# MSNLAB/Federated-Lifelong-Person-ReID

Hardware: AMD Instinct MI355X
Metric: images/sec (whole node) per fed round, fedstil resnet50 (higher is better)
Workload: dtype bf16; 1 GPU; model=resnet50-fedstil, global_batch=64, img=128x64, images_per_round_per_client=512, num_classes=8000, lambda_k=2000, rehearsal_set=2000 exemplar budget + task (m=32/id), parallelism=fed-dp1 (1 client/GPU)

## Files before the change

flreid_amd/methods/common.py:

```python

from __future__ import annotations

import collections
import os
from typing import Any, Dict, List, Optional, Union

import torch
from torch.utils.data import DataLoader

from flreid_amd import ops
from flreid_amd.modules.client import ClientModule
from flreid_amd.modules.operator import OperatorModule
from flreid_amd.runtime.precision import autocast
from flreid_amd.tools.evaluate import calculate_similarity_distance, evaluate
from flreid_amd.tools.utils import model_on_device


def reset_optimizer_state_inplace(optimizer) -> None:
    import collections

    for state in optimizer.state.values():
        zeroed = True
        for k, v in state.items():
            if torch.is_tensor(v):
                v.zero_()
            elif isinstance(v, (int, float)):
                zeroed = False
        if not zeroed:
            optimizer.state = collections.defaultdict(dict)
            return


class BaseReIDOperator(OperatorModule):

    def set_optimizer_parameters(self, model, capturable: bool = False) -> None:
        defaults = dict(self.optimizer.defaults)
        if capturable and "capturable" in defaults:
            defaults["capturable"] = True
        params = [p for p in model.net.parameters() if p.requires_grad]
        for p in params:
            state = self.optimizer.state.get(p)
            if state and any(torch.is_tensor(v) and v.dim() > 0
                             and v.shape != p.shape for v in state.values()):
                del self.optimizer.state[p]
        group = {"params": params, **defaults}
        if capturable:
            group["capturable"] = True
        if (isinstance(self.optimizer, (torch.optim.Adam, torch.optim.AdamW))
                and params and params[0].is_cuda
                and os.environ.get("FLREID_FUSED_ADAM", "1") == "1"):
            group["fused"] = True
            group["foreach"] = False
        self.optimizer.param_groups = [group]

    def penalty(self, model) -> Optional[torch.Tensor]:
        return None

    def train_forward(self, model, data, target, **kwargs) -> Dict:
        score, feature = model.forward(data)
        loss = 0.0
        for loss_func in self.criterion:
            loss = loss + loss_func(score=score, feature=feature, target=target)
        return {"score": score, "feature": feature, "loss": loss}

    _invoke_train = train_forward
    _invoke_predict = train_forward

    def invoke_train(self, model, dataloader: DataLoader, **kwargs) -> Any:
        train_acc = train_loss = 0.0
        batch_cnt = data_cnt = 0
        device = model.device

        model.train()
        acc_dev = loss_dev = None
        for data, person_id, _classes_id in dataloader:
            data = data.to(device, non_blocking=True)
            target = person_id.to(device, non_blocking=True)
            self.optimizer.zero_grad(set_to_none=True)
            with autocast(device):
                output = self.train_forward(model, data, target, **kwargs)
                loss = output["loss"]
                pen = self.penalty(model)
                if pen is not None:
                    loss = loss + pen
            loss.backward()
            self.optimizer.step()
            score = output["score"]
            b_acc = (score.detach().argmax(dim=1) == target).sum()
            b_loss = loss.detach()
            acc_dev = b_acc if acc_dev is None else acc_dev + b_acc
            loss_dev = b_loss if loss_dev is None else loss_dev + b_loss
            data_cnt += len(data)
            batch_cnt += 1
        if acc_dev is not None:
            train_acc = float(acc_dev)
            train_loss = float(loss_dev)

        train_acc /= max(1, data_cnt)
        train_loss /= max(1, batch_cnt)
        if self.scheduler:
            self.scheduler.step()
        return {"accuracy": train_acc, "loss": train_loss,
                "batch_count": batch_cnt, "data_count": data_cnt}

    def invoke_predict(self, model, dataloader: DataLoader, **kwargs) -> Any:
        pred_acc = pred_loss = 0.0
        batch_cnt = data_cnt = 0
        device = model.device

        model.train()
        for data, person_id, _classes_id in dataloader:
            data, target = data.to(device), person_id.to(device)
            with torch.no_grad(), autocast(device):
                output = self.train_forward(model, data, target, **kwargs)
            pred_acc += (output["score"].argmax(dim=1) == target).sum().item()
            pred_loss += float(output["loss"])
            data_cnt += len(data)
            batch_cnt += 1
        return {"accuracy": pred_acc / max(1, data_cnt),
                "loss": pred_loss / max(1, batch_cnt),
                "batch_count": batch_cnt, "data_count": data_cnt}

    def _eval_features(self, model, dataloader: DataLoader, collect_labels: bool):
        device = model.device
        feats, labels = [], []
        batch_cnt = data_cnt = 0
        model.eval()
        for data, person_id, _classes_id in dataloader:
            data = data.to(device, non_blocking=True)
            with torch.no_grad(), autocast(device):
                feat = model.forward(data)
            feat = ops.l2_normalize(feat.float(), dim=1)
            feats.append(feat.detach())
            if collect_labels:
                labels.append(person_id.clone().detach())
            data_cnt += len(data)
            batch_cnt += 1
        feats = torch.cat(feats, dim=0).cpu() if feats else torch.empty(0)
        out = {"features": feats, "batch_count": batch_cnt, "data_count": data_cnt}
        if collect_labels:
            out["labels"] = torch.cat(labels, dim=0) if labels else torch.empty(0, dtype=torch.long)
        return out

    def invoke_valid(self, model, dataloader: DataLoader, **kwargs) -> Any:
        return self._eval_features(model, dataloader, collect_labels=True)

    def invoke_inference(self, model, dataloader: DataLoader, **kwargs) -> Any:
        return self._eval_features(model, dataloader, collect_labels=False)

    def _invoke_valid(self, model, data, target, **kwargs):
        feat = model.forward(data)
        return {"feature": ops.l2_normalize(feat, dim=1)}

    def _invoke_inference(self, model, data, **kwargs):
        feat = model.forward(data)
        return {"feature": ops.l2_normalize(feat, dim=1)}


class BaseReIDClient(ClientModule):

    default_ckpt_name: str = "model"

    def __init__(self, client_name, model, operator, ckpt_root,
                 model_ckpt_name=None, **kwargs):
        super().__init__(client_name, model, operator, ckpt_root,
                         model_ckpt_name, **kwargs)
        if not self.model_ckpt_name:
            self.model_ckpt_name = self.default_ckpt_name
        self.train_cnt = 0
        self.test_cnt = 0

    def before_task_train(self, task_name: str, tr_loader) -> None:
        pass

    def after_task_train(self, output: Dict, tr_loader, device: str) -> None:
        pass

    def train(self, epochs: int, task_name: str,
              tr_loader: Union[List[DataLoader], DataLoader],
              val_loader: Union[List[DataLoader], DataLoader],
              early_stop_threshold: int = 3, device: str = "cpu",
              **kwargs) -> Any:
        self.load_model(self.model_ckpt_name)
        self.before_task_train(task_name, tr_loader)

        output: Dict = {}
        perf_loss, perf_acc, sustained_cnt = 1e8, 0.0, 0
        initial_lr = self.operator.optimizer.defaults["lr"]

        with model_on_device(self.model, device):
            for epoch in range(1, epochs + 1):
                output = self.train_one_epoch(task_name, tr_loader, val_loader)
                accuracy, loss = output["accuracy"], output["loss"]
                data_count = output["data_count"]

                sustained_cnt += 1
                if loss <= perf_loss and accuracy >= perf_acc:
                    perf_loss, perf_acc = loss, accuracy
                    sustained_cnt = 0
                if early_stop_threshold and sustained_cnt >= early_stop_threshold:
                    break

                self.train_cnt += data_count
                self.logger.info_train(task_name, device, data_count,
                                       perf_acc, perf_loss, epoch, epochs)
            self.after_task_train(output, tr_loader, device)

        reset_optimizer_state_inplace(self.operator.optimizer)
        for group in self.operator.optimizer.param_groups:
            group["lr"] = initial_lr

        self.save_model(self.model_ckpt_name)
        return output

    def train_one_epoch(self, task_name, tr_loader, val_loader, **kwargs) -> Any:
        return self.operator.invoke_train(self.model, tr_loader)

    def inference(self, task_name, query_loader, gallery_loader,
                  device: str = "cpu", **kwargs) -> Any:
        self.load_model(self.model_ckpt_name)
        with model_on_device(self.model, device):
            gallery_features = self.operator.invoke_inference(self.model, gallery_loader)["features"]
            query_features = self.operator.invoke_inference(self.model, query_loader)["features"]
        self.test_cnt += len(gallery_features) + len(query_features)

        output = {}
        for query_id in range(len(query_features)):
            sims = calculate_similarity_distance(query_features[query_id], gallery_features)
            output[query_id] = {gid: d for gid, d in enumerate(sims)}
        return output

    def validate(self, task_name, query_loader, gallery_loader,
                 device: str = "cpu", **kwargs) -> Any:
        self.load_model(self.model_ckpt_name)
        with model_on_device(self.model, device):
            gallery_output = self.operator.invoke_valid(self.model, gallery_loader)
            query_output = self.operator.invoke_valid(self.model, query_loader)

        gallery_size = len(gallery_output["features"])
        query_size = len(query_output["features"])
        self.test_cnt += gallery_size + query_size

        cmc, mAP = evaluate(
            query_features=query_output["features"],
            query_labels=query_output["labels"],
            gallery_features=gallery_output["features"],
            gallery_labels=gallery_output["labels"],
            device=device,
        )
        avg_rep = torch.cat([query_output["features"], gallery_output["features"]], dim=0)
        avg_rep = avg_rep.sum(dim=0) / len(avg_rep)
        self.logger.info_validation(task_name, query_size, gallery_size, cmc, mAP)
        return cmc, mAP, avg_rep


def weighted_average_states(states: Dict[str, Dict], key: str,
                            counts: Dict[str, int]) -> Dict[str, torch.Tensor]:
    total = sum(counts.values())
    merged: Dict[str, torch.Tensor] = {}
    for cname, cstate in states.items():
        k = counts[cname]
        if total == 0:
            continue
        for n, p in cstate[key].items():
            contrib = p.detach().to(torch.float32) * (k / total)
            if n not in merged:
                merged[n] = torch.zeros_like(contrib)
            merged[n] += contrib
    out = {}
    for cname, cstate in states.items():
        for n, p in cstate[key].items():
            if n in merged and n not in out:
                out[n] = merged[n].to(p.dtype)
    return out
```

flreid_amd/methods/fedstil.py:

```python

from __future__ import annotations

import math
from typing import Any, Dict, List, Optional

import torch
from torch.utils.data import DataLoader

from flreid_amd import ops
from flreid_amd.methods.common import BaseReIDClient, BaseReIDOperator
from flreid_amd.models.adaptive import (
    adaptive_leaves,
    convert_to_adaptive,
    non_adaptive_leaves,
)
from flreid_amd.modules.model import ModelModule
from flreid_amd.modules.server import ServerModule
from flreid_amd.runtime.precision import autocast
from flreid_amd.tools.distance import compute_kl_distance


class Model(ModelModule):

    atten_trainable = False

    def __init__(self, net, lambda_l1: float = 1e-4, lambda_k: int = 8000,
                 atten_default: float = 0.80, **kwargs):
        super().__init__(net)
        self.lambda_l1 = lambda_l1
        self.lambda_k = lambda_k
        self.atten_default = atten_default
        self.args = kwargs

        self._convert_net()

        self.ids = set()
        self.examplars: Dict[int, List] = {}
        self.examplars_nhwc = False
        self._egraphs: Dict = {}

        leaves = adaptive_leaves(self.net)
        if not leaves:
            raise ValueError("fedstil requires at least one trainable "
                             "Linear/Conv2d (check fine_tuning)")
        self.head_stage = min(self.net.stage_of(n) for n, _ in leaves)

    def _convert_net(self) -> None:
        convert_to_adaptive(self.net, self.atten_default,
                            atten_trainable=self.atten_trainable)

    def adaptive_module_leaves(self):
        return adaptive_leaves(self.net)

    def pre_trained_module_leaves(self):
        return non_adaptive_leaves(self.net)

    def eval_graphed(self, key: str, fn, data: torch.Tensor, full: bool):
        from flreid_amd.runtime.hipgraph import GraphedStep, hipgraph_enabled
        if (not full or not hipgraph_enabled()
                or not str(data.device).startswith("cuda")):
            return fn(data)
        cache_key = (key, tuple(data.shape))
        gs = self._egraphs.get(cache_key)
        if gs is None:
            gs = GraphedStep(lambda d: (fn(d),))
            gs.warmup(data)
            out = gs.capture(data)
            self._egraphs[cache_key] = gs
            return out[0]
        return gs(data)[0]

    def head_forward(self, head_input: torch.Tensor):
        out, _ = self.net.run_stages(head_input, start=self.head_stage)
        return out

    def tap_forward(self, data: torch.Tensor):
        out, tap = self.net.run_stages(data, start=0, tap=self.head_stage)
        return out, tap

    def forward(self, data: torch.Tensor) -> Any:
        return self.net(data)

    @property
    def m(self) -> int:
        return math.ceil(self.lambda_k / max(1, len(self.ids)))

    def examplar_tensors(self, device, nhwc: Optional[bool] = None):
        if not self.examplars:
            return None, None, None
        if nhwc is not None and nhwc != self.examplars_nhwc:
            perm = (0, 2, 3, 1) if nhwc else (0, 3, 1, 2)
            for pid in list(self.examplars):
                protos_t, classes_t = self.examplars[pid]
                if protos_t.dim() == 4:
                    self.examplars[pid] = (
                        protos_t.permute(*perm).contiguous(), classes_t)
            self.examplars_nhwc = nhwc
        datas, pids, classes = [], [], []
        for pid, entry in self.examplars.items():
            protos_t, classes_t = entry
            datas.append(protos_t.to(device))
            pids.append(torch.full((protos_t.shape[0],), int(pid), dtype=torch.long))
            classes.append(classes_t)
        return torch.cat(datas), torch.cat(pids), torch.cat(classes)

    @torch.no_grad()
    def build_examplars(self, proto_loader, person_ids, device) -> None:
        self.eval()
        stacked = getattr(proto_loader, "data", None)
        if torch.is_tensor(stacked):
            protos = stacked.to(device)
            if protos.shape[0] == 0:
                return
            pids = proto_loader.pids
            classes = proto_loader.classes
            feats = []
            chunk = 512
            present = getattr(proto_loader, "present", lambda t: t)
            for i in range(0, protos.shape[0], chunk):
                rows = protos[i:i + chunk]
                nrow = rows.shape[0]
                if nrow < chunk and str(device).startswith("cuda"):
                    rows = torch.cat([rows, protos.new_zeros(
                        (chunk - nrow, *protos.shape[1:]))])
                data = present(rows)
                with autocast(device):
                    sf = self.eval_graphed("herd_fwd", self.head_forward, data,
                                           full=data.shape[0] == chunk)
                feat = sf[1] if isinstance(sf, tuple) else sf
                feats.append(feat[:nrow].float())
            feats = torch.cat(feats)
        else:
            protos, pids, classes, feats = [], [], [], []
            bsz = getattr(proto_loader, "batch_size", None)
            for data, person_id, class_id in proto_loader:
                data = data.to(device)
                with autocast(device):
                    _score_feat = self.eval_graphed(
                        "herd_fwd", self.head_forward, data,
                        full=data.shape[0] == bsz)
                feature = _score_feat[1] if isinstance(_score_feat, tuple) \
                    else _score_feat
                protos.append(data)
                pids.append(person_id)
                classes.append(class_id)
                feats.append(feature.float())
            if not protos:
                return
            protos = torch.cat(protos)
            pids = torch.cat(pids)
            classes = torch.cat(classes)
            feats = torch.cat(feats)

        if person_ids is not None and len(person_ids):
            allowed = torch.as_tensor([int(x) for x in person_ids],
                                      dtype=pids.dtype)
            keep = torch.isin(pids, allowed)
            protos, pids, classes, feats = protos[keep.to(protos.device)], \
                pids[keep], classes[keep], feats[keep.to(feats.device)]

        dev = feats.device
        order = torch.argsort(pids, stable=True)
        persons_t, counts_t = torch.unique_consecutive(
            pids[order], return_counts=True)
        persons = persons_t.tolist()
        P = len(persons)
        nmax = int(counts_t.max())
        D = feats.shape[1]
        offsets = torch.cat([torch.zeros(1, dtype=torch.long),
                             counts_t.cumsum(0)[:-1]])
        pos = torch.arange(pids.numel()) - offsets.repeat_interleave(counts_t)
        group = torch.arange(P).repeat_interleave(counts_t)

        order_dev = order.to(dev)
        f_pad = torch.zeros(P, nmax, D, device=dev)
        f_pad[group.to(dev), pos.to(dev)] = feats.index_select(0, order_dev)
        pad_penalty = torch.zeros(P, nmax, device=dev)
        pad_mask = pos.new_zeros(P, nmax, dtype=torch.bool)
        pad_mask[group, pos] = True
        pad_penalty.masked_fill_(~pad_mask.to(dev), 1e30)
        counts = counts_t.to(dev, torch.float32)
        mu = f_pad.sum(dim=1) / counts.unsqueeze(1)

        fsq = (f_pad * f_pad).sum(dim=2)
        acc = torch.zeros(P, D, device=dev)
        arange_p = torch.arange(P, device=dev)
        step_idx = []
        for i in range(self.m):
            g = mu * (i + 1) - acc
            dots = torch.bmm(f_pad, g.unsqueeze(2)).squeeze(2)
            score = fsq - 2.0 * dots + pad_penalty
            idx = score.argmin(dim=1)
            step_idx.append(idx)
            acc = acc + f_pad[arange_p, idx]
        sel = torch.stack(step_idx, dim=1).cpu()

        chosen = order.view(-1)[(offsets.unsqueeze(1) + sel).clamp_max(
            pids.numel() - 1).view(-1)].view(P, -1)
        proto_sel = protos.index_select(
            0, chosen.view(-1).to(protos.device)).view(P, -1, *protos.shape[1:])
        class_sel = classes.index_select(0, chosen.view(-1)).view(P, -1)
        for r, p in enumerate(persons):
            self.examplars[int(p)] = (proto_sel[r], class_sel[r])
        if torch.is_tensor(stacked):
            self.examplars_nhwc = bool(getattr(proto_loader, "nhwc_stored",
                                               False))

    def reduce_examplars(self) -> None:
        for k in list(self.examplars):
            protos_t, classes_t = self.examplars[k]
            self.examplars[k] = (protos_t[:self.m], classes_t[:self.m])

    def model_state(self) -> Dict:
        leaves = self.adaptive_module_leaves()
        state = {
            "global_weight": {f"{n}.global_weight": l.global_weight.detach().clone()
                              for n, l in leaves},
            "global_weight_atten": {f"{n}.global_weight_atten":
                                    l.global_weight_atten.detach().clone()
                                    for n, l in leaves},
            "adaptive_weights": {f"{n}.adaptive_weight":
                                 l.adaptive_weight.detach().clone()
                                 for n, l in leaves},
            "adaptive_bias": {f"{n}.adaptive_bias": l.adaptive_bias.detach().clone()
                              for n, l in leaves if l.adaptive_bias is not None},
            "bn_params": {},
            "pre_trained_params": {
                f"{ln}.{pn}": p.detach().clone()
                for ln, layer in self.pre_trained_module_leaves()
                for pn, p in layer.state_dict().items()
            },
        }
        return state

    def update_model(self, params_state: Dict) -> None:
        live = {n: t for n, t in self.net.state_dict(keep_vars=True).items()}
        rebound = False
        with torch.no_grad():
            for section in ("global_weight", "global_weight_atten",
                            "adaptive_weights", "adaptive_bias", "bn_params",
                            "pre_trained_params"):
                for n, p in params_state.get(section, {}).items():
                    dst = live.get(n)
                    if dst is None:
                        continue
                    if dst.shape == p.shape:
                        dst.copy_(p.detach(), non_blocking=True)
                    else:
                        mod = self.net.get_submodule(n.rsplit(".", 1)[0])
                        leaf = n.rsplit(".", 1)[1]
                        target = getattr(mod, leaf)
                        target.data = p.detach().clone().to(dst.device, dst.dtype)
                        if hasattr(target, "grad"):
                            target.grad = None
                        rebound = True
        if rebound:
            self._egraphs.clear()

    def composed_upload(self) -> Dict[str, torch.Tensor]:
        return {f"{n}.global_weight": l.composed_weight().detach().clone()
                for n, l in self.adaptive_module_leaves()}

    def drift_loss(self) -> torch.Tensor:
        pairs = []
        for _n, l in self.adaptive_module_leaves():
            pairs.extend(l.drift_pairs())
        return ops.l1_drift(pairs)


class TensorBatches:

    def __init__(self, data: torch.Tensor, pids: torch.Tensor,
                 classes: torch.Tensor, batch_size: int, shuffle: bool = True,
                 nhwc_stored: bool = False):
        self.data, self.pids, self.classes = data, pids, classes
        self.batch_size = batch_size
        self.shuffle = shuffle
        self.nhwc_stored = nhwc_stored
        self._pids_dev = pids.to(data.device) if data.is_cuda else None
        n = data.shape[0]
        self.drop_last = n % batch_size == 1
        self._len = n // batch_size + (0 if (self.drop_last or n % batch_size == 0) else 1)

    def present(self, rows: torch.Tensor) -> torch.Tensor:
        if self.nhwc_stored and rows.dim() == 4:
            return rows.permute(0, 3, 1, 2)
        return rows

    def __len__(self):
        return self._len

    def __iter__(self):
        n = self.data.shape[0]
        order_cpu = torch.randperm(n) if self.shuffle else torch.arange(n)
        order_dev = order_cpu.to(self.data.device, non_blocking=True)
        stop = self._len * self.batch_size if self.drop_last else n
        for i in range(0, stop, self.batch_size):
            idx_cpu = order_cpu[i:i + self.batch_size]
            idx_dev = order_dev[i:i + self.batch_size]
            pid_sel = (self._pids_dev.index_select(0, idx_dev)
                       if self._pids_dev is not None
                       else self.pids.index_select(0, idx_cpu))
            yield (self.present(self.data.index_select(0, idx_dev)),
                   pid_sel,
                   self.classes.index_select(0, idx_cpu))


class Operator(BaseReIDOperator):
    def generate_proto_loader(self, model: Model, source_loader: DataLoader):
        device = model.device
        model.eval()
        on_gpu = str(device).startswith("cuda")
        with torch.no_grad():
            if on_gpu:
                datas, pids, classes = [], [], []
                for data, person_id, class_id in source_loader:
                    datas.append(data.to(device, non_blocking=True))
                    pids.append(person_id)
                    classes.append(class_id)
                data_all = torch.cat(datas)
                taps = []
                chunk = 512
                for i in range(0, data_all.shape[0], chunk):
                    d = data_all[i:i + chunk]
                    nrow = d.shape[0]
                    if nrow < chunk:
                        d = torch.cat([d, data_all.new_zeros(
                            (chunk - nrow, *data_all.shape[1:]))])
                    with autocast(device):
                        tap = model.eval_graphed(
                            "tap_fwd", lambda t: model.tap_forward(t)[1], d,
                            full=d.shape[0] == chunk)
                    tap = tap[:nrow]
                    taps.append((tap.permute(0, 2, 3, 1) if tap.dim() == 4
                                 else tap).clone())
                del data_all, datas
            else:
                taps, pids, classes = [], [], []
                bsz = getattr(source_loader, "batch_size", None)
                for data, person_id, class_id in source_loader:
                    data = data.to(device, non_blocking=True)
                    with autocast(device):
                        tap = model.eval_graphed(
                            "tap_fwd", lambda d: model.tap_forward(d)[1], data,
                            full=data.shape[0] == bsz)
                    taps.append(tap.float())
                    pids.append(person_id)
                    classes.append(class_id)
        taps = torch.cat(taps)
        pids = torch.cat(pids)
        classes = torch.cat(classes)

        ex_data, ex_pids, ex_classes = model.examplar_tensors(
            device, nhwc=on_gpu and taps.dim() == 4)
        if ex_data is not None:
            all_data = torch.cat([ex_data, taps])
            all_pids = torch.cat([ex_pids, pids])
            all_classes = torch.cat([ex_classes, classes])
        else:
            all_data, all_pids, all_classes = taps, pids, classes

        loader = TensorBatches(all_data, all_pids, all_classes,
                               source_loader.batch_size, shuffle=True,
                               nhwc_stored=on_gpu and all_data.dim() == 4)
        task_token = taps.reshape(taps.shape[0], -1).mean(
            dim=0, dtype=torch.float32).cpu()
        return loader, task_token

    def _train_step(self, model: Model, data: torch.Tensor,
                    target: torch.Tensor):
        device = model.device
        self.optimizer.zero_grad(set_to_none=True)
        with autocast(device):
            score, feature = model.head_forward(data)
            loss = 0.0
            for loss_func in self.criterion:
                loss = loss + loss_func(score=score, feature=feature, target=target)
            loss = loss + model.drift_loss() * model.lambda_l1
        loss.backward()
        self.optimizer.step()
        b_acc = (score.detach().argmax(dim=1) == target).sum()
        return loss.detach(), b_acc

    def _graphed_step(self, model: Model, batch_size: int):
        from flreid_amd.runtime.hipgraph import GraphedStep

        lr = self.optimizer.param_groups[0]["lr"]
        shapes = tuple(tuple(p.shape) for p in
                       self.optimizer.param_groups[0]["params"])
        key = (batch_size, float(lr), shapes)
        cache = getattr(self, "_train_graphs", None)
        if cache is None or cache[0] != key:
            gs = GraphedStep(lambda d, t: self._train_step(model, d, t))
            self._train_graphs = (key, gs)
        return self._train_graphs[1]

    def _epoch_graph(self, model: Model, loader) -> "EpochGraph":
        from flreid_amd.runtime.hipgraph import EpochGraph

        n, batch = loader.data.shape[0], loader.batch_size
        steps = n // batch
        lr = float(self.optimizer.param_groups[0]["lr"])
        shapes = tuple(tuple(p.shape) for p in
                       self.optimizer.param_groups[0]["params"])
        key = (tuple(loader.data.shape), batch, steps, lr, shapes)
        cache = getattr(self, "_epoch_graph_cache", None)
        if cache is None or cache[0] != key:
            eg = EpochGraph(lambda d, t: self._train_step(model, d, t),
                            steps, batch, loader.data, loader._pids_dev,
                            loader.present)
            self._epoch_graph_cache = (key, eg)
        return self._epoch_graph_cache[1]

    def invoke_train(self, model: Model, dataloader: DataLoader, **kwargs) -> Any:
        from flreid_amd.runtime.hipgraph import epoch_graph_enabled, hipgraph_enabled

        train_acc = train_loss = 0.0
        batch_cnt = data_cnt = 0
        device = model.device
        use_graph = hipgraph_enabled() and str(device).startswith("cuda")
        from flreid_amd.runtime.hipgraph import phase
        with phase("proto_capture"):
            proto_loader, task_token = self.generate_proto_loader(model, dataloader)

        model.train()
        self.set_optimizer_parameters(model, capturable=use_graph)
        batch_size = getattr(proto_loader, "batch_size", None)
        _phase_head = phase("head_epoch"); _phase_head.__enter__()

        use_epoch = (use_graph and epoch_graph_enabled()
                     and isinstance(proto_loader, TensorBatches)
                     and proto_loader.data.is_cuda
                     and proto_loader._pids_dev is not None
                     and proto_loader.data.shape[0] >= batch_size)
        if use_epoch:
            n = proto_loader.data.shape[0]
            steps = n // batch_size
            order = torch.randperm(n)
            eg = self._epoch_graph(model, proto_loader)
            idx_flat = order[:steps * batch_size].to(device, non_blocking=True)
            loss_dev, acc_dev = eg.run(proto_loader.data,
                                       proto_loader._pids_dev, idx_flat)
            batch_cnt, data_cnt = steps, steps * batch_size
            stop = (steps * batch_size
                    if (proto_loader.drop_last or n % batch_size == 0) else n)
            if stop > steps * batch_size:
                tail = order[steps * batch_size:stop].to(device)
                d = proto_loader.present(
                    proto_loader.data.index_select(0, tail))
                t = proto_loader._pids_dev.index_select(0, tail)
                b_loss, b_acc = self._train_step(model, d, t)
                loss_dev = loss_dev + b_loss
                acc_dev = acc_dev + b_acc
                batch_cnt += 1
                data_cnt += tail.numel()
        else:
            gs = self._graphed_step(model, batch_size) if use_graph else None
            warmups = 0

            acc_dev = loss_dev = None
            for data, person_id, _class_id in proto_loader:
                data = data.to(device, non_blocking=True)
                target = person_id.to(device, non_blocking=True)
                if gs is not None and data.shape[0] == batch_size:
                    if gs.ready:
                        b_loss, b_acc = gs(data, target)
                    elif warmups < 2:
                        b_loss, b_acc = gs.warmup(data, target)
                        warmups += 1
                    else:
                        b_loss, b_acc = gs.capture(data, target)
                else:
                    b_loss, b_acc = self._train_step(model, data, target)
                acc_dev = b_acc.clone() if acc_dev is None else acc_dev + b_acc
                loss_dev = b_loss.clone() if loss_dev is None else loss_dev + b_loss
                data_cnt += len(data)
                batch_cnt += 1
        _phase_head.__exit__(None, None, None)
        if acc_dev is not None:
            train_acc = float(acc_dev)
            train_loss = float(loss_dev)

        if self.scheduler:
            self.scheduler.step()
        return {
            "task_token": task_token,
            "proto_loader": proto_loader,
            "accuracy": train_acc / max(1, data_cnt),
            "loss": train_loss / max(1, batch_cnt),
            "batch_count": batch_cnt,
            "data_count": data_cnt,
        }


class Client(BaseReIDClient):
    default_ckpt_name = "fedstil_model"

    def __init__(self, client_name, model: Model, operator, ckpt_root,
                 model_ckpt_name=None, **kwargs):
        super().__init__(client_name, model, operator, ckpt_root,
                         model_ckpt_name, **kwargs)
        self.current_task: Optional[str] = None
        self.task_token: Optional[torch.Tensor] = None

    @staticmethod
    def _examplars_to_ckpt(examplars: Dict, nhwc: bool = False) -> Dict:
        out = {}
        for pid, (protos_t, classes_t) in examplars.items():
            if nhwc and protos_t.dim() == 4:
                protos_t = protos_t.permute(0, 3, 1, 2)
            out[pid] = [(protos_t[i].cpu(), int(classes_t[i]))
                        for i in range(protos_t.shape[0])]
        return out

    @staticmethod
    def _examplars_from_ckpt(ck: Dict) -> Dict:
        out = {}
        for pid, items in ck.items():
            if isinstance(items, tuple):
                out[pid] = items
                continue
            protos = torch.stack([p for p, _c in items]) if items else torch.empty(0)
            classes = torch.tensor([c for _p, c in items], dtype=torch.long)
            out[pid] = (protos, classes)
        return out

    def load_model(self, model_name: str) -> None:
        if self.state_exists(model_name):
            self.model.update_model(self.load_state(model_name, None))
        if self.state_exists(f"{model_name}_examplars"):
            self.model.examplars = self._examplars_from_ckpt(
                self.load_state(f"{model_name}_examplars", {}))
            self.model.examplars_nhwc = False

    def save_model(self, model_name: str) -> None:
        if self._ckpt_disabled():
            return
        self.save_state(model_name, self.model.model_state(), True)
        self.save_state(f"{model_name}_examplars",
                        self._examplars_to_ckpt(self.model.examplars,
                                                self.model.examplars_nhwc),
                        True)

    def update_model(self, params_state: Dict) -> None:
        self.model.update_model(params_state)

    def get_incremental_state(self, **kwargs) -> Dict:
        return {
            "train_cnt": self.train_cnt,
            "task_token": self.task_token,
            "incremental_sw": self.model.composed_upload(),
            "incremental_bn": self.model.model_state()["bn_params"],
        }

    def get_integrated_state(self, **kwargs) -> Dict:
        state = self.model.model_state()
        return {
            "train_cnt": self.train_cnt,
            "task_token": self.task_token,
            "integrated_sw": self.model.composed_upload(),
            "integrated_bn": state["bn_params"],
            "pre_trained_params": state["pre_trained_params"],
        }

    def _reload_then(self, params: Dict) -> None:
        if self.current_task:
            self.load_model(self.model_ckpt_name or self.current_task)
        self.update_model(params)
        for _n, layer in self.model.adaptive_module_leaves():
            layer.init_training_weights()

    def update_by_incremental_state(self, state: Dict, **kwargs) -> Any:
        self._reload_then({"global_weight": state["incremental_shared_params"]})

    def update_by_integrated_state(self, state: Dict, **kwargs) -> Any:
        self._reload_then({
            "global_weight": state["integrated_global_weight"],
            "bn_params": state["integrated_bn_params"],
            "pre_trained_params": state["integrated_pre_trained_params"],
        })

    def train(self, epochs, task_name, tr_loader, val_loader,
              early_stop_threshold: int = 3, device: str = "cpu", **kwargs) -> Any:
        import collections

        if self.current_task is None or self.current_task != task_name:
            self.model.ids.update(int(p) for p in tr_loader.dataset.person_ids)
        self.current_task = task_name

        output: Dict = {}
        perf_loss, perf_acc, sustained_cnt = 1e8, 0.0, 0
        initial_lr = self.operator.optimizer.defaults["lr"]
        task_tokens = []

        from flreid_amd.tools.utils import model_on_device
        with model_on_device(self.model, device):
            for epoch in range(1, epochs + 1):
                output = self.train_one_epoch(task_name, tr_loader, val_loader)
                accuracy, loss = output["accuracy"], output["loss"]

                sustained_cnt += 1
                if loss <= perf_loss and accuracy >= perf_acc:
                    perf_loss, perf_acc = loss, accuracy
                    sustained_cnt = 0
                if early_stop_threshold and sustained_cnt >= early_stop_threshold:
                    break

                task_tokens.append(output["task_token"])
                self.train_cnt += output["data_count"]
                self.logger.info_train(task_name, device, output["data_count"],
                                       perf_acc, perf_loss, epoch, epochs)

            from flreid_amd.runtime.hipgraph import phase
            self.model.reduce_examplars()
            with phase("herding"):
                self.model.build_examplars(output["proto_loader"],
                                           tr_loader.dataset.person_ids, device)

        from flreid_amd.methods.common import reset_optimizer_state_inplace
        reset_optimizer_state_inplace(self.operator.optimizer)
        for group in self.operator.optimizer.param_groups:
            group["lr"] = initial_lr

        if task_tokens:
            self.task_token = sum(task_tokens) / len(task_tokens)

        self.save_model(self.model_ckpt_name or self.current_task)
        return output

    def validate(self, task_name, query_loader, gallery_loader,
                 device: str = "cpu", **kwargs) -> Any:
        if not self.model_ckpt_name:
            self.model_ckpt_name = task_name
        return super().validate(task_name, query_loader, gallery_loader,
                                device, **kwargs)


class Server(ServerModule):
    def __init__(self, server_name, model: Model, operator, ckpt_root,
                 distance_calculate_step: int = 10,
                 distance_calculate_decay: float = 0.8, **kwargs):
        super().__init__(server_name, model, operator, ckpt_root, **kwargs)
        self.token_memory: Dict[str, List[torch.Tensor]] = {}
        self.distance_calculate_step = distance_calculate_step
        self.distance_calculate_decay = distance_calculate_decay

    def update_model(self, params_state: Dict) -> None:
        self.model.update_model(params_state)

    def load_model(self, model_name: str) -> None:
        self.model.update_model(self.load_state(model_name, self.model.model_state()))

    def save_model(self, model_name: str) -> None:
        import os as _os
        if _os.environ.get("FLREID_DISABLE_CKPT", "0") == "1":
            return
        self.save_state(model_name, self.model.model_state(), True)

    def calculate(self) -> Any:
        states = {c: s for c, s in self.clients.items() if s}
        if not states:
            return
        total = sum(s["train_cnt"] for s in states.values())
        if total == 0:
            return
        merged: Dict[str, torch.Tensor] = {}
        for _c, s in states.items():
            k = s["train_cnt"]
            for n, p in s["incremental_sw"].items():
                contrib = p.detach().to(torch.float32) * (k / total)
                merged[n] = merged.get(n, 0) + contrib
        self.model.update_model({"global_weight": merged})
        self.save_state(f"{self.server_name}_tokens", self.token_memory, True)

    def _remember_token(self, client_name: str, state: Dict) -> None:
        if state.get("task_token") is not None:
            self.token_memory.setdefault(client_name, []).append(state["task_token"])

    def set_client_incremental_state(self, client_name: str, client_state: Dict) -> None:
        if client_name not in self.clients:
            self.logger.warn(f"unregistered client {client_name} upload ignored")
            return
        self.clients[client_name] = client_state
        self._remember_token(client_name, client_state)

    def set_client_integrated_state(self, client_name: str, client_state: Dict) -> None:
        self.set_client_incremental_state(client_name, client_state)

    def get_dispatch_incremental_state(self, client_name: str) -> Dict:
        own_state = self.clients.get(client_name)
        if own_state is None or own_state.get("task_token") is None:
            return {"incremental_shared_params": self.model.model_state()["global_weight"]}

        task_token = own_state["task_token"].unsqueeze(0)
        select_client, token_distance = [], []
        for c_name, c_tokens in self.token_memory.items():
            if c_name == client_name:
                continue
            c_tokens = c_tokens[::-1 * self.distance_calculate_step]
            dis = 1e-8
            for decay_cnt, other_token in enumerate(c_tokens):
                d = compute_kl_distance(task_token, other_token.unsqueeze(0))
                dis += float(d) / math.pow(self.distance_calculate_decay, decay_cnt)
            select_client.append(c_name)
            token_distance.append(1.0 / dis)

        select_client.append(client_name)
        token_distance.append(sum(token_distance) / len(token_distance)
                              if token_distance else 1.0)

        total = sum(token_distance)
        token_distance = [d / total for d in token_distance]
        token_distance = torch.softmax(torch.tensor(token_distance), dim=0).tolist()

        merged: Dict[str, torch.Tensor] = {}
        for c_name, mix in zip(select_client, token_distance):
            params = self.clients[c_name]["incremental_sw"]
            for n, p in params.items():
                contrib = p.detach().to(torch.float32) * mix
                merged[n] = merged.get(n, 0) + contrib
        merged = {n: p for n, p in merged.items()}
        return {"incremental_shared_params": merged}

    def get_dispatch_integrated_state(self, client_name: str) -> Dict:
        state = self.model.model_state()
        return {
            "integrated_global_weight": state["global_weight"],
            "integrated_bn_params": state["bn_params"],
            "integrated_pre_trained_params": state["pre_trained_params"],
        }
```

flreid_amd/models/adaptive.py:

```python

from __future__ import annotations

import os
from typing import Optional, Tuple

import torch
import torch.nn.functional as F
from torch import nn
from torch.nn import Parameter

from flreid_amd import ops


class AdaptiveBase(nn.Module):

    def __init__(self, global_weight: torch.Tensor,
                 global_weight_atten: Optional[torch.Tensor] = None,
                 adaptive_weight: Optional[torch.Tensor] = None,
                 adaptive_bias: Optional[torch.Tensor] = None,
                 atten_default: float = 0.80, atten_trainable: bool = False,
                 **kwargs):
        super().__init__()
        self.atten_default = atten_default
        self.atten_trainable = atten_trainable
        self.global_weight = Parameter(torch.empty(0), requires_grad=False)
        self.global_weight_atten = Parameter(torch.empty(0), requires_grad=False)
        self.adaptive_weight = Parameter(torch.empty(0))
        self.adaptive_bias = Parameter(torch.empty(0)) if adaptive_bias is not None else None
        self.initial_global_weight_atten = Parameter(torch.empty(0), requires_grad=False)
        self.initial_adaptive_weight = Parameter(torch.empty(0), requires_grad=False)
        self.init_training_weights(global_weight, global_weight_atten,
                                   adaptive_weight, adaptive_bias)

    @staticmethod
    def _assign(param: Parameter, value: torch.Tensor) -> None:
        if param.data.shape == value.shape:
            param.data.copy_(value)
        else:
            param.data = value.detach().clone().to(param.device)
            param.grad = None

    @torch.no_grad()
    def init_training_weights(self, global_weight=None, global_weight_atten=None,
                              adaptive_weight=None, adaptive_bias=None) -> None:
        if global_weight is None:
            global_weight = self.global_weight.data
        self._assign(self.global_weight, global_weight.detach())
        self.global_weight.requires_grad = False

        if global_weight_atten is None:
            global_weight_atten = torch.ones(
                self.global_weight.data.shape[-1],
                device=self.global_weight.device) * self.atten_default
        self._assign(self.global_weight_atten, global_weight_atten.detach())
        self._assign(self.initial_global_weight_atten, global_weight_atten.detach())
        self.global_weight_atten.requires_grad = self.atten_trainable

        if adaptive_weight is None:
            adaptive_weight = (1.0 - self.global_weight_atten.data) * self.global_weight.data
        self._assign(self.adaptive_weight, adaptive_weight.detach())
        self._assign(self.initial_adaptive_weight, adaptive_weight.detach())
        self.adaptive_weight.requires_grad = True

        if self.adaptive_bias is not None and adaptive_bias is not None:
            self._assign(self.adaptive_bias, adaptive_bias.detach())
            self.adaptive_bias.requires_grad = True

    def composed_weight(self) -> torch.Tensor:
        return ops.adaptive_compose(self.global_weight, self.global_weight_atten,
                                    self.adaptive_weight)

    def drift_pairs(self):
        return [(self.global_weight_atten, self.initial_global_weight_atten),
                (self.adaptive_weight, self.initial_adaptive_weight)]


class AdaptiveLinear(AdaptiveBase):
    def forward(self, data: torch.Tensor) -> torch.Tensor:
        if data.dim() == 2:
            return ops.adaptive_linear(data, self.global_weight,
                                       self.global_weight_atten,
                                       self.adaptive_weight,
                                       self.adaptive_bias)
        return F.linear(data, self.composed_weight(), self.adaptive_bias)


def _is_one(v) -> bool:
    return v == 1 or v == (1, 1) or v == [1, 1]


def _is_zero(v) -> bool:
    return v == 0 or v == (0, 0) or v == [0, 0]


class AdaptiveConv2d(AdaptiveBase):
    def __init__(self, global_weight, stride=1, padding=0, **kwargs):
        super().__init__(global_weight, **kwargs)
        self.stride = stride
        self.padding = padding

    def forward(self, data: torch.Tensor) -> torch.Tensor:
        gw = self.global_weight
        if (data.is_cuda and gw.dim() == 4 and gw.shape[2] == 3
                and gw.shape[3] == 3 and _is_one(self.stride)
                and _is_one(self.padding) and self.adaptive_bias is None
                and not gw.requires_grad
                and not self.global_weight_atten.requires_grad):
            y = ops.conv3x3_try(data, gw, self.global_weight_atten,
                                self.adaptive_weight)
            if y is not None:
                return y
        if (data.is_cuda and gw.dim() == 4 and gw.shape[2] == 1
                and gw.shape[3] == 1 and _is_one(self.stride)
                and _is_zero(self.padding)):
            b, c, h, w = data.shape
            n_out = gw.shape[0]
            xv = data.permute(0, 2, 3, 1).reshape(-1, c)
            y = None
            if not gw.requires_grad and not self.global_weight_atten.requires_grad:
                aw2d = self.adaptive_weight.view(n_out, c) \
                    if self.adaptive_weight.numel() else None
                y = ops.adaptive_linear_1x1(xv, gw.view(n_out, c),
                                            self.global_weight_atten, aw2d,
                                            self.adaptive_bias)
            if y is None:
                theta = self.composed_weight().view(n_out, c)
                y = F.linear(xv, theta, self.adaptive_bias)
            return y.view(b, h, w, -1).permute(0, 3, 1, 2)
        return F.conv2d(data, self.composed_weight(), self.adaptive_bias,
                        stride=self.stride, padding=self.padding)


class AdaptiveBatchNorm2d(AdaptiveBase):

    def __init__(self, global_weight, running_mean=None, running_var=None,
                 num_batches_tracked=None, track_running_stats=False,
                 momentum=0.1, eps=1e-5, **kwargs):
        super().__init__(global_weight, **kwargs)
        self.register_buffer("running_mean", running_mean)
        self.register_buffer("running_var", running_var)
        self.register_buffer("num_batches_tracked", num_batches_tracked)
        self.track_running_stats = track_running_stats
        self.momentum = momentum
        self.eps = eps

    def forward(self, data: torch.Tensor) -> torch.Tensor:
        training = self.training or (self.running_mean is None and self.running_var is None)
        use_stats = not self.training or self.track_running_stats
        return F.batch_norm(
            data,
            self.running_mean if use_stats else None,
            self.running_var if use_stats else None,
            self.composed_weight(), self.adaptive_bias,
            training, self.momentum or 0.0, self.eps)


class AdaptiveLayerNorm(AdaptiveBase):
    def __init__(self, global_weight, normalized_shape: Tuple[int, ...] = None,
                 eps: float = 1e-5, **kwargs):
        super().__init__(global_weight, **kwargs)
        self.normalized_shape = normalized_shape or tuple(global_weight.shape)
        self.eps = eps

    def forward(self, data: torch.Tensor) -> torch.Tensor:
        return F.layer_norm(data, self.normalized_shape, self.composed_weight(),
                            self.adaptive_bias, self.eps)


ADAPTIVE_TYPES = (AdaptiveLinear, AdaptiveConv2d, AdaptiveBatchNorm2d, AdaptiveLayerNorm)


def convert_to_adaptive(net: nn.Module, atten_default: float = 0.80,
                        atten_trainable: bool = False) -> int:
    count = 0
    for name, module in list(net.named_modules()):
        if isinstance(module, (nn.Linear, nn.Conv2d)):
            if not all(p.requires_grad for p in module.parameters()):
                continue
            if isinstance(module, nn.Linear):
                new = AdaptiveLinear(
                    global_weight=module.weight, adaptive_bias=module.bias,
                    atten_default=atten_default, atten_trainable=atten_trainable)
            else:
                new = AdaptiveConv2d(
                    global_weight=module.weight, adaptive_bias=module.bias,
                    atten_default=atten_default, atten_trainable=atten_trainable,
                    stride=module.stride, padding=module.padding)
            parent = net
            parts = name.split(".")
            for p in parts[:-1]:
                parent = getattr(parent, p)
            setattr(parent, parts[-1], new)
            count += 1
    return count


def adaptive_leaves(net: nn.Module):
    return [(n, m) for n, m in net.named_modules() if isinstance(m, ADAPTIVE_TYPES)]


def non_adaptive_leaves(net: nn.Module):
    out = []
    for n, m in net.named_modules():
        if len(list(m.children())) == 0 and not isinstance(m, ADAPTIVE_TYPES) and n:
            out.append((n, m))
    return out



class StackedAttenBase(nn.Module):

    def __init__(self, global_weight: torch.Tensor,
                 adaptive_bias: Optional[torch.Tensor] = None,
                 atten_default: float = 0.0, **kwargs):
        super().__init__()
        self.atten_default = atten_default
        self.atten_trainable = True
        self.global_weight = Parameter(torch.empty(0), requires_grad=False)
        self.global_weight_atten = Parameter(torch.empty(0))
        self.adaptive_weight = Parameter(torch.empty(0))
        self.adaptive_bias = Parameter(torch.empty(0)) if adaptive_bias is not None else None
        self.initial_global_weight_atten = Parameter(torch.empty(0), requires_grad=False)
        self.initial_adaptive_weight = Parameter(torch.empty(0), requires_grad=False)
        self.init_training_weights(global_weight.unsqueeze(-1),
                                   adaptive_bias=adaptive_bias)

    _assign = staticmethod(AdaptiveBase._assign)

    @torch.no_grad()
    def init_training_weights(self, global_weight=None, global_weight_atten=None,
                              adaptive_weight=None, adaptive_bias=None) -> None:
        if global_weight is None:
            global_weight = self.global_weight.data
        self._assign(self.global_weight, global_weight.detach())
        self.global_weight.requires_grad = False

        k = self.global_weight.shape[-1]
        if global_weight_atten is None:
            global_weight_atten = torch.ones(k, device=self.global_weight.device) \
                                  * self.atten_default
        self._assign(self.global_weight_atten, global_weight_atten.detach())
        self._assign(self.initial_global_weight_atten, global_weight_atten.detach())
        self.global_weight_atten.requires_grad = True

        if self.adaptive_weight.numel() == 0:
            if adaptive_weight is None:
                adaptive_weight = ((1.0 - self.global_weight_atten.data)
                                   * self.global_weight.data).sum(dim=-1)
            self._assign(self.adaptive_weight, adaptive_weight.detach())
        elif adaptive_weight is not None:
            self._assign(self.adaptive_weight, adaptive_weight.detach())
        self.adaptive_weight.requires_grad = True
        self._assign(self.initial_adaptive_weight, self.adaptive_weight.detach())

        if self.adaptive_bias is not None and adaptive_bias is not None:
            self._assign(self.adaptive_bias, adaptive_bias.detach())
            self.adaptive_bias.requires_grad = True

    def composed_weight(self) -> torch.Tensor:
        return (self.global_weight_atten * self.global_weight).sum(dim=-1) \
               + self.adaptive_weight

    def drift_pairs(self):
        return [(self.global_weight_atten, self.initial_global_weight_atten),
                (self.adaptive_weight, self.initial_adaptive_weight)]


class StackedAttenLinear(StackedAttenBase):
    def forward(self, data: torch.Tensor) -> torch.Tensor:
        return F.linear(data, self.composed_weight(), self.adaptive_bias)


class StackedAttenConv2d(StackedAttenBase):
    def __init__(self, global_weight, stride=1, padding=0, **kwargs):
        super().__init__(global_weight, **kwargs)
        self.stride = stride
        self.padding = padding

    def forward(self, data: torch.Tensor) -> torch.Tensor:
        return F.conv2d(data, self.composed_weight(), self.adaptive_bias,
                        stride=self.stride, padding=self.padding)


ADAPTIVE_TYPES = ADAPTIVE_TYPES + (StackedAttenLinear, StackedAttenConv2d)


def convert_to_stacked(net: nn.Module, atten_default: float = 0.0) -> int:
    count = 0
    for name, module in list(net.named_modules()):
        if isinstance(module, (nn.Linear, nn.Conv2d)):
            if not all(p.requires_grad for p in module.parameters()):
                continue
            if isinstance(module, nn.Linear):
                new = StackedAttenLinear(global_weight=module.weight,
                                         adaptive_bias=module.bias,
                                         atten_default=atten_default)
            else:
                new = StackedAttenConv2d(global_weight=module.weight,
                                         adaptive_bias=module.bias,
                                         atten_default=atten_default,
                                         stride=module.stride,
                                         padding=module.padding)
            parent = net
            parts = name.split(".")
            for p in parts[:-1]:
                parent = getattr(parent, p)
            setattr(parent, parts[-1], new)
            count += 1
    return count
```

flreid_amd/ops/__init__.py:

```python

from __future__ import annotations

import os
from typing import Dict, Optional

import torch

from flreid_amd.ops import reference as ref

_EXT = None
_EXT_ERR: Optional[str] = None

_F32, _BF16 = 0, 1


def _load_extension():
    global _EXT, _EXT_ERR
    if _EXT is not None or _EXT_ERR is not None:
        return _EXT
    try:
        from flreid_amd.ops import _flreid_hip

        _EXT = _flreid_hip
    except Exception as e:
        _EXT_ERR = f"{type(e).__name__}: {e}"
        _EXT = None
    return _EXT


def extension_available() -> bool:
    return _load_extension() is not None


def _ext_or_raise(opname: str):
    ext = _load_extension()
    if ext is not None:
        return ext
    if os.environ.get("FLREID_ALLOW_EAGER", "0") == "1":
        return None
    raise RuntimeError(
        f"flreid HIP extension missing for GPU op '{opname}' ({_EXT_ERR}). "
        "Build it with `python -m flreid_amd.ops.build` "
        "or set FLREID_ALLOW_EAGER=1 to debug with eager PyTorch."
    )


def _stream() -> int:
    return torch.cuda.current_stream().cuda_stream


def _dt(t: torch.Tensor) -> int:
    if t.dtype == torch.float32:
        return _F32
    if t.dtype == torch.bfloat16:
        return _BF16
    raise TypeError(f"unsupported dtype {t.dtype}")



def _pairwise_gpu(ext, a: torch.Tensor, b: torch.Tensor, mode: int) -> torch.Tensor:
    a = a.contiguous().float()
    b = b.contiguous().float()
    m, n, d = a.shape[0], b.shape[0], a.shape[1]
    out = torch.empty(m, n, device=a.device, dtype=torch.float32)
    if mode == 2:
        aa = torch.empty(m, device=a.device, dtype=torch.float32)
        bb = torch.empty(n, device=a.device, dtype=torch.float32)
        ext.rowsq(a.data_ptr(), aa.data_ptr(), m, d, _stream())
        ext.rowsq(b.data_ptr(), bb.data_ptr(), n, d, _stream())
    else:
        aa = bb = out
    ext.pairwise(a.data_ptr(), b.data_ptr(), aa.data_ptr(), bb.data_ptr(),
                 out.data_ptr(), m, n, d, mode, _stream())
    return out


def similarity_matrix(a: torch.Tensor, b: torch.Tensor) -> torch.Tensor:
    if a.is_cuda and not a.requires_grad and not b.requires_grad:
        ext = _ext_or_raise("pairwise")
        if ext is not None:
            return _pairwise_gpu(ext, a, b, 0)
    return a.float() @ b.float().t()


def pairwise_sqeuclidean(a: torch.Tensor, b: torch.Tensor) -> torch.Tensor:
    if a.is_cuda and not a.requires_grad and not b.requires_grad:
        ext = _ext_or_raise("pairwise")
        if ext is not None:
            return _pairwise_gpu(ext, a, b, 2)
    return ref.pairwise_sqeuclidean(a, b)


def pairwise_cosine_distance(a: torch.Tensor, b: torch.Tensor) -> torch.Tensor:
    if a.is_cuda and not a.requires_grad and not b.requires_grad:
        ext = _ext_or_raise("pairwise")
        if ext is not None:
            return _pairwise_gpu(ext, l2_normalize(a.float()),
                                 l2_normalize(b.float()), 1)
    return ref.pairwise_cosine_distance(a, b)



def l2_normalize(x: torch.Tensor, dim: int = 1) -> torch.Tensor:
    if (x.is_cuda and x.dim() == 2 and dim in (1, -1)
            and not x.requires_grad and x.dtype in (torch.float32, torch.bfloat16)):
        ext = _ext_or_raise("l2norm_rows")
        if ext is not None:
            x = x.contiguous()
            y = torch.empty_like(x)
            ext.l2norm_rows(x.data_ptr(), y.data_ptr(), x.shape[0], x.shape[1],
                            _dt(x), 1e-12, _stream())
            return y
    return ref.l2_normalize(x, dim=dim)



class _CeLabelSmoothFn(torch.autograd.Function):
    @staticmethod
    def forward(ctx, score, target, epsilon, ext):
        score_c = score.contiguous()
        B, C = score_c.shape
        row_loss = torch.empty(B, device=score.device, dtype=torch.float32)
        grad = torch.empty_like(score_c)
        ext.ce_smooth(score_c.data_ptr(), target.contiguous().data_ptr(),
                      row_loss.data_ptr(), grad.data_ptr(), B, C,
                      _dt(score_c), float(epsilon), _stream())
        ctx.save_for_backward(grad)
        return row_loss.sum() * (1.0 / B)

    @staticmethod
    def backward(ctx, grad_out):
        (grad,) = ctx.saved_tensors
        return grad * grad_out, None, None, None


def ce_label_smooth(score: torch.Tensor, target: torch.Tensor,
                    epsilon: float = 0.1) -> torch.Tensor:
    if score.is_cuda and score.dim() == 2:
        ext = _ext_or_raise("ce_smooth")
        if ext is not None:
            return _CeLabelSmoothFn.apply(score, target.long(), epsilon, ext)
    return ref.ce_label_smooth(score, target, epsilon)



class _ComposeFn(torch.autograd.Function):

    @staticmethod
    def forward(ctx, gw, atten, aw, ext):
        gw_c, aw_c = gw.contiguous(), aw.contiguous()
        at = atten.detach().contiguous().float()
        out = torch.empty_like(gw_c)
        ext.compose(gw_c.data_ptr(), at.data_ptr(), aw_c.data_ptr(),
                    out.data_ptr(), gw_c.numel(), gw_c.shape[-1], _dt(gw_c),
                    _stream())
        ctx.atten_requires = atten.requires_grad
        if ctx.atten_requires:
            ctx.save_for_backward(gw_c)
        return out

    @staticmethod
    def backward(ctx, grad_out):
        g_atten = None
        if ctx.atten_requires:
            (gw,) = ctx.saved_tensors
            g_atten = (grad_out * gw).reshape(-1, gw.shape[-1]).sum(dim=0)
        return None, g_atten, grad_out, None


def adaptive_compose(global_weight: torch.Tensor, atten: torch.Tensor,
                     adaptive_weight: torch.Tensor) -> torch.Tensor:
    if (global_weight.is_cuda and not global_weight.requires_grad
            and global_weight.dtype in (torch.float32, torch.bfloat16)
            and adaptive_weight.dtype == global_weight.dtype):
        ext = _ext_or_raise("compose")
        if ext is not None:
            return _ComposeFn.apply(global_weight, atten, adaptive_weight, ext)
    return ref.adaptive_compose(global_weight, atten, adaptive_weight)



_TORCH_DT = {torch.float32: _F32, torch.bfloat16: _BF16}


def _decomposed_geometry(sw: torch.Tensor):
    rows = sw.shape[0]
    if sw.dim() == 4:
        c, s = sw.shape[1], sw.shape[2] * sw.shape[3]
        if s > 1 and c > 1 and not sw.is_contiguous():
            if sw.is_contiguous(memory_format=torch.channels_last):
                return rows, c, s, True
            return None
        if sw.is_contiguous() or sw.is_contiguous(
                memory_format=torch.channels_last):
            return rows, c, s, False
        return None
    if not sw.is_contiguous():
        return None
    return rows, sw.numel() // max(rows, 1), 1, False


class _DecomposedComposeFn(torch.autograd.Function):

    @staticmethod
    def forward(ctx, sw, mask, aw, aw_kb, atten, lambda_l1, lambda_mask,
                training, out_dtype, geom, ext):
        rows, c, s, cl = geom
        kb = aw_kb.shape[-1]
        out = torch.empty_like(sw, dtype=out_dtype)
        ext.decomposed_fwd(sw.data_ptr(), mask.data_ptr(), aw.data_ptr(),
                           aw_kb.data_ptr(), atten.data_ptr(), out.data_ptr(),
                           rows, c, s, kb, int(cl), int(training),
                           float(lambda_l1), float(lambda_mask),
                           _TORCH_DT[out_dtype], _stream())
        ctx.save_for_backward(sw, mask, aw, aw_kb, atten)
        ctx.cfg = (geom, float(lambda_l1), float(lambda_mask), bool(training),
                   out_dtype, ext)
        return out

    @staticmethod
    def backward(ctx, grad_out):
        sw, mask, aw, aw_kb, atten = ctx.saved_tensors
        (rows, c, s, cl), l1, lm, training, out_dtype, ext = ctx.cfg
        need_mask, need_aw, need_atten = (ctx.needs_input_grad[1],
                                          ctx.needs_input_grad[2],
                                          ctx.needs_input_grad[4])
        if not (need_mask or need_aw or need_atten):
            return (None,) * 11
        kb = aw_kb.shape[-1]
        g = grad_out.to(out_dtype)
        g = g.contiguous(memory_format=torch.channels_last) if cl \
            else g.contiguous()
        tpr, blocks = ext.decomposed_plan(rows, c, s, int(cl))
        dev = sw.device
        d_aw = torch.empty_like(aw) if need_aw else None
        dm_part = (torch.empty(rows, tpr, device=dev, dtype=torch.float32)
                   if need_mask else None)
        da_part = (torch.empty(blocks, kb, device=dev, dtype=torch.float32)
                   if need_atten else None)
        ext.decomposed_bwd(
            g.data_ptr(), _TORCH_DT[out_dtype], sw.data_ptr(),
            mask.data_ptr(), aw.data_ptr(), aw_kb.data_ptr(),
            d_aw.data_ptr() if need_aw else 0,
            dm_part.data_ptr() if need_mask else 0,
            da_part.data_ptr() if need_atten else 0,
            rows, c, s, kb, int(cl), int(training), l1, lm,
            int(need_aw), int(need_mask), int(need_atten), _stream())
        d_mask = dm_part.sum(dim=1).view(mask.shape) if need_mask else None
        d_atten = da_part.sum(dim=0).view(atten.shape) if need_atten else None
        return (None, d_mask, d_aw, None, d_atten) + (None,) * 6


def decomposed_compose(sw: torch.Tensor, mask: torch.Tensor, aw: torch.Tensor,
                       aw_kb: torch.Tensor, atten: torch.Tensor,
                       lambda_l1: float, lambda_mask: float, training: bool,
                       out_dtype: Optional[torch.dtype] = None) -> torch.Tensor:
    if (sw.is_cuda and os.environ.get("FLREID_NO_FUSED_DECOMPOSE", "0") != "1"
            and out_dtype in (None, torch.float32, torch.bfloat16)
            and all(t.is_cuda and t.dtype == torch.float32
                    for t in (sw, mask, aw, aw_kb, atten))
            and sw.dim() >= 2 and sw.numel() > 0 and not sw.requires_grad
            and not aw_kb.requires_grad and aw.shape == sw.shape
            and aw_kb.dim() == sw.dim() + 1 and aw_kb.shape[:-1] == sw.shape
            and aw_kb.shape[-1] >= 1 and aw_kb.is_contiguous()
            and atten.numel() == aw_kb.shape[-1] and atten.is_contiguous()
            and mask.numel() == sw.shape[0] and mask.is_contiguous()):
        geom = _decomposed_geometry(sw)
        if geom is not None and geom == _decomposed_geometry(aw):
            ext = _ext_or_raise("decomposed_fwd")
            if ext is not None:
                return _DecomposedComposeFn.apply(
                    sw, mask, aw, aw_kb, atten, lambda_l1, lambda_mask,
                    bool(training), out_dtype or torch.float32, geom, ext)
    out = ref.decomposed_compose(sw, mask, aw, aw_kb, atten, lambda_l1,
                                 lambda_mask, training)
    if out_dtype is not None and out.dtype != out_dtype:
        out = out.to(out_dtype)
    return out



def importance_update(importance: Dict[str, torch.Tensor],
                      grads: Dict[str, torch.Tensor], mode: str = "sq",
                      scale: float = 1.0) -> None:
    first = next(iter(importance.values()), None)
    if first is not None and first.is_cuda:
        ext = _ext_or_raise("importance")
        if ext is not None:
            for n, g in grads.items():
                if g is None:
                    continue
                F = importance[n]
                ext.importance(F.data_ptr(), g.contiguous().data_ptr(),
                               g.numel(), _dt(g), mode == "sq", scale,
                               _stream())
            return
    for n, g in grads.items():
        if g is None:
            continue
        if mode == "sq":
            importance[n] += (g.detach().float() ** 2) * scale
        else:
            importance[n] += g.detach().float().abs() * scale



kl_distance = ref.kl_distance
quadratic_penalty = ref.quadratic_penalty
l1_drift_fused = ref.l1_drift_fused


class _KdLossFn(torch.autograd.Function):

    @staticmethod
    def forward(ctx, zs, zt, temperature, ext):
        zs_c = zs.detach().float().contiguous()
        zt_c = zt.detach().float().contiguous()
        B, C = zs_c.shape
        row_loss = torch.empty(B, device=zs.device, dtype=torch.float32)
        grad = torch.empty_like(zs_c)
        ext.kd_fwd(zs_c.data_ptr(), zt_c.data_ptr(), row_loss.data_ptr(),
                   grad.data_ptr(), B, C, float(temperature), _stream())
        ctx.save_for_backward(grad)
        ctx.zs_dtype = zs.dtype
        return row_loss.sum()

    @staticmethod
    def backward(ctx, grad_out):
        (grad,) = ctx.saved_tensors
        return (grad * grad_out).to(ctx.zs_dtype), None, None, None


def kd_loss(logits_student: torch.Tensor, logits_teacher: torch.Tensor,
            temperature: float = 4.0) -> torch.Tensor:
    if logits_student.is_cuda and logits_student.dim() == 2:
        ext = _ext_or_raise("kd_fwd")
        if ext is not None:
            return _KdLossFn.apply(logits_student, logits_teacher,
                                   temperature, ext)
    return ref.kd_loss(logits_student, logits_teacher, temperature)


class _IcarlDistillFn(torch.autograd.Function):

    @staticmethod
    def forward(ctx, score, target, prev, ext):
        score_c = score.detach().float().contiguous()
        prev_c = prev.detach().float().contiguous()
        B, C = score_c.shape
        P = prev_c.shape[1]
        row_loss = torch.empty(B, device=score.device, dtype=torch.float32)
        grad = torch.empty_like(score_c)
        ext.icarl_distill(score_c.data_ptr(),
                          target.long().contiguous().data_ptr(),
                          prev_c.data_ptr(), row_loss.data_ptr(),
                          grad.data_ptr(), B, C, P, _stream())
        ctx.save_for_backward(grad)
        ctx.score_dtype = score.dtype
        return row_loss.sum()

    @staticmethod
    def backward(ctx, grad_out):
        (grad,) = ctx.saved_tensors
        return (grad * grad_out).to(ctx.score_dtype), None, None, None


def icarl_distill_loss(score: torch.Tensor, target: torch.Tensor,
                       prev_logits: torch.Tensor) -> torch.Tensor:
    if (score.is_cuda and score.dim() == 2
            and prev_logits.shape[1] <= score.shape[1]):
        ext = _ext_or_raise("icarl_distill")
        if ext is not None:
            return _IcarlDistillFn.apply(score, target, prev_logits, ext)
    return ref.icarl_distill_loss(score, target, prev_logits)


class _TripletHardFn(torch.autograd.Function):

    @staticmethod
    def forward(ctx, feature, target, margin, ext):
        f = feature.detach().contiguous().float()
        n, d = f.shape
        norms = torch.empty(n, device=f.device, dtype=torch.float32)
        ext.rowsq(f.data_ptr(), norms.data_ptr(), n, d, _stream())
        row_loss = torch.empty(n, device=f.device, dtype=torch.float32)
        p_idx = torch.empty(n, device=f.device, dtype=torch.int32)
        n_idx = torch.empty(n, device=f.device, dtype=torch.int32)
        ext.triplet_fwd(f.data_ptr(), norms.data_ptr(),
                        target.contiguous().data_ptr(), row_loss.data_ptr(),
                        p_idx.data_ptr(), n_idx.data_ptr(), n, d,
                        float(margin), _stream())
        ctx.save_for_backward(f, row_loss, p_idx, n_idx)
        ctx.ext = ext
        return row_loss.mean()

    @staticmethod
    def backward(ctx, grad_out):
        f, row_loss, p_idx, n_idx = ctx.saved_tensors
        n, d = f.shape
        grad = torch.zeros_like(f)
        coeff = float(grad_out) * 2.0 / n
        ctx.ext.triplet_bwd(f.data_ptr(), row_loss.data_ptr(),
                            p_idx.data_ptr(), n_idx.data_ptr(),
                            grad.data_ptr(), n, d, coeff, _stream())
        return grad, None, None, None


def triplet_loss(feature: torch.Tensor, target: torch.Tensor,
                 margin: Optional[float] = 0.3, norm_feat: bool = False,
                 hard_mining: bool = True) -> torch.Tensor:
    if (feature.is_cuda and hard_mining and not norm_feat
            and margin is not None and margin > 0 and feature.dim() == 2):
        ext = _ext_or_raise("triplet_fwd")
        if ext is not None:
            return _TripletHardFn.apply(feature.float(), target.long(),
                                        margin, ext)
    return ref.triplet_loss(feature, target, margin, norm_feat, hard_mining)


def cmc_map(query_features, query_labels, gallery_features, gallery_labels,
            query_camera_labels=None, gallery_camera_labels=None,
            query_chunk: int = 2048):
    if not query_features.is_cuda:
        return ref.cmc_map(query_features, query_labels, gallery_features,
                           gallery_labels, query_camera_labels,
                           gallery_camera_labels)
    q = query_features.shape[0]
    g = gallery_features.shape[0]
    if q <= query_chunk:
        sims = similarity_matrix(query_features, gallery_features)
        return ref.cmc_map_from_sims(sims, query_labels, gallery_labels,
                                     query_camera_labels, gallery_camera_labels)
    total_cmc = torch.zeros(g, dtype=torch.float64)
    total_ap = 0.0
    for s0 in range(0, q, query_chunk):
        s1 = min(q, s0 + query_chunk)
        sims = similarity_matrix(query_features[s0:s1], gallery_features)
        cmc, mAP = ref.cmc_map_from_sims(
            sims, query_labels[s0:s1], gallery_labels,
            query_camera_labels[s0:s1] if query_camera_labels is not None else None,
            gallery_camera_labels)
        n = s1 - s0
        total_cmc += cmc * n
        total_ap += mAP * n
    return total_cmc / q, total_ap / q


def _window_attn_fwd_raw(ext, q, k, v, bias, mask, scale):
    bw, h, n, d = q.shape
    qc, kc, vc = q.contiguous(), k.contiguous(), v.contiguous()
    bias_c = bias.detach().contiguous().float()
    if mask is not None:
        mask_c = mask.detach().contiguous().float()
        nw = mask_c.shape[0]
        mask_ptr = mask_c.data_ptr()
    else:
        mask_c, nw, mask_ptr = None, 1, 0
    out = torch.empty_like(qc)
    ext.window_attn_fwd(qc.data_ptr(), kc.data_ptr(), vc.data_ptr(),
                        bias_c.data_ptr(), mask_ptr, out.data_ptr(),
                        bw, h, n, d, nw, float(scale), _dt(qc), _stream())
    return out, qc, kc, vc, bias_c, mask_c


class _WindowAttnFn(torch.autograd.Function):

    @staticmethod
    def forward(ctx, q, k, v, bias, mask, scale):
        ext = _ext_or_raise("window_attn_fwd")
        out, qc, kc, vc, bias_c, mask_c = _window_attn_fwd_raw(
            ext, q.detach(), k.detach(), v.detach(), bias, mask, scale)
        ctx.save_for_backward(qc, kc, vc, bias_c)
        ctx.mask_c = mask_c
        ctx.scale = float(scale)
        ctx.bias_requires = bias.requires_grad
        return out

    @staticmethod
    def backward(ctx, grad_out):
        ext = _ext_or_raise("window_attn_bwd")
        qc, kc, vc, bias_c = ctx.saved_tensors
        mask_c = ctx.mask_c
        bw, h, n, d = qc.shape
        nw = mask_c.shape[0] if mask_c is not None else 1
        go = grad_out.contiguous().to(qc.dtype)
        dq = torch.empty_like(qc)
        dk = torch.empty_like(kc)
        dv = torch.empty_like(vc)
        ds = torch.empty(bw, h, n, n, device=qc.device, dtype=torch.float32)
        ext.window_attn_bwd(qc.data_ptr(), kc.data_ptr(), vc.data_ptr(),
                            bias_c.data_ptr(),
                            mask_c.data_ptr() if mask_c is not None else 0,
                            go.data_ptr(), dq.data_ptr(), dk.data_ptr(),
                            dv.data_ptr(), ds.data_ptr(), bw, h, n, d, nw,
                            ctx.scale, _dt(qc), _stream())
        dbias = ds.sum(dim=0) if ctx.bias_requires else None
        return dq, dk, dv, dbias, None, None


def window_attention(q, k, v, bias, mask, scale, dropout=None):
    drop_p = 0.0
    if dropout is not None:
        drop_p = float(getattr(dropout, "p", 0.0))
    if (q.is_cuda and q.shape[-2] <= 64 and q.shape[-1] <= 64
            and drop_p == 0.0 and extension_available()):
        if not torch.is_grad_enabled():
            ext = _ext_or_raise("window_attn_fwd")
            out, *_ = _window_attn_fwd_raw(ext, q, k, v, bias, mask, scale)
            return out
        return _WindowAttnFn.apply(q, k, v, bias, mask, scale)
    return ref.window_attention(q, k, v, bias, mask, scale, dropout)


class _PatchMergeLNFn(torch.autograd.Function):

    @staticmethod
    def forward(ctx, x, gamma, beta, H, W, eps):
        ext = _ext_or_raise("patch_merge_ln_fwd")
        x_c = x.detach().contiguous()
        b, L, c = x_c.shape
        rows = b * (H // 2) * (W // 2)
        y = torch.empty(b, L // 4, 4 * c, device=x.device, dtype=x.dtype)
        mean = torch.empty(rows, device=x.device, dtype=torch.float32)
        rstd = torch.empty(rows, device=x.device, dtype=torch.float32)
        gamma_c = gamma.detach().float().contiguous()
        beta_c = beta.detach().float().contiguous()
        ext.patch_merge_ln_fwd(x_c.data_ptr(), gamma_c.data_ptr(),
                               beta_c.data_ptr(), y.data_ptr(),
                               mean.data_ptr(), rstd.data_ptr(), rows, c, H,
                               W, float(eps), _dt(x_c), _stream())
        ctx.save_for_backward(x_c, gamma_c, mean, rstd)
        ctx.hw = (H, W)
        return y

    @staticmethod
    def backward(ctx, dy):
        ext = _ext_or_raise("patch_merge_ln_bwd")
        x_c, gamma_c, mean, rstd = ctx.saved_tensors
        H, W = ctx.hw
        b, L, c = x_c.shape
        rows = b * (H // 2) * (W // 2)
        nblk = (rows + 3) // 4
        dy_c = dy.contiguous().to(x_c.dtype)
        dx = torch.empty_like(x_c)
        dg_part = torch.empty(nblk, 4 * c, device=x_c.device,
                              dtype=torch.float32)
        db_part = torch.empty(nblk, 4 * c, device=x_c.device,
                              dtype=torch.float32)
        ext.patch_merge_ln_bwd(x_c.data_ptr(), gamma_c.data_ptr(),
                               dy_c.data_ptr(), mean.data_ptr(),
                               rstd.data_ptr(), dx.data_ptr(),
                               dg_part.data_ptr(), db_part.data_ptr(), rows,
                               c, H, W, _dt(x_c), _stream())
        dgamma = dg_part.sum(0) if ctx.needs_input_grad[1] else None
        dbeta = db_part.sum(0) if ctx.needs_input_grad[2] else None
        return dx, dgamma, dbeta, None, None, None


def patch_merge_ln(x: torch.Tensor, gamma: torch.Tensor, beta: torch.Tensor,
                   H: int, W: int, eps: float = 1e-5) -> Optional[torch.Tensor]:
    if (not x.is_cuda or x.dim() != 3 or H % 2 or W % 2
            or 4 * x.shape[2] > 3072 or x.shape[1] != H * W
            or not extension_available()):
        return None
    if x.dtype not in (torch.float32, torch.bfloat16):
        return None
    return _PatchMergeLNFn.apply(x, gamma, beta, H, W, eps)


def adaptive_linear_fwd(x: torch.Tensor, gw: torch.Tensor,
                        atten: Optional[torch.Tensor],
                        aw: Optional[torch.Tensor],
                        bias: Optional[torch.Tensor],
                        split_layout: int = 1) -> torch.Tensor:
    ext = _ext_or_raise("adaptive_linear_fwd")
    if ext is None:
        theta = ref.adaptive_compose(gw, atten, aw) if atten is not None else gw
        return (torch.nn.functional.linear(x.float(), theta,
                                           bias).to(x.dtype))
    m, k = x.shape
    n = gw.shape[0]
    x_c = x.contiguous()
    out = torch.empty(m, n, device=x.device, dtype=torch.bfloat16)
    ext.adaptive_linear_fwd(
        x_c.data_ptr(), gw.contiguous().data_ptr(),
        aw.contiguous().data_ptr() if aw is not None else 0,
        atten.contiguous().float().data_ptr() if atten is not None else 0,
        bias.contiguous().float().data_ptr() if bias is not None else 0,
        out.data_ptr(), m, n, k, split_layout, _stream())
    return out


class _AdaptiveLinearFn(torch.autograd.Function):

    @staticmethod
    def forward(ctx, x, gw, atten, aw, bias):
        x_bf = x.detach().to(torch.bfloat16).contiguous()
        out = adaptive_linear_fwd(x_bf, gw.detach(), atten, aw.detach(),
                                  bias.detach() if bias is not None else None)
        ctx.save_for_backward(x_bf, gw, atten, aw)
        ctx.has_bias = bias is not None
        ctx.x_dtype = x.dtype
        return out

    @staticmethod
    def backward(ctx, grad_out):
        x_bf, gw, atten, aw = ctx.saved_tensors
        g = grad_out.to(torch.bfloat16)
        ext = _load_extension()
        if ext is not None and gw.dtype == torch.float32:
            theta = compose_theta_bf16(ext, gw.contiguous(), atten,
                                       aw.contiguous())
        else:
            theta = adaptive_compose(gw, atten, aw).to(torch.bfloat16)
        grad_x = (g @ theta).to(ctx.x_dtype)
        grad_aw = (g.t() @ x_bf).to(aw.dtype)
        grad_bias = grad_out.sum(0).to(torch.float32) if ctx.has_bias else None
        return grad_x, None, None, grad_aw, grad_bias


def adaptive_linear(x: torch.Tensor, gw: torch.Tensor, atten: torch.Tensor,
                    aw: torch.Tensor, bias: Optional[torch.Tensor]):
    if (x.is_cuda and x.dim() == 2 and not gw.requires_grad
            and not atten.requires_grad and gw.shape[-1] % 32 == 0
            and atten.numel() == gw.shape[-1]
            and extension_available()):
        return _AdaptiveLinearFn.apply(x, gw, atten, aw, bias)
    theta = adaptive_compose(gw, atten, aw)
    return torch.nn.functional.linear(x, theta, bias)


def bn_eval_2d(x: torch.Tensor, bn, relu: bool = False) -> Optional[torch.Tensor]:
    if (not x.is_cuda or x.requires_grad or bn.running_mean is None
            or x.dtype not in (torch.float32, torch.bfloat16)
            or x.dim() not in (2, 4)):
        return None
    ext = _load_extension()
    if ext is None:
        return None
    if x.dim() == 2:
        if not x.is_contiguous():
            x = x.contiguous()
        nhwc, hw = True, 1
    else:
        nhwc = x.is_contiguous(memory_format=torch.channels_last)
        if not nhwc and not x.is_contiguous():
            x = x.contiguous()
        hw = x.shape[2] * x.shape[3]
    out = torch.empty_like(x)
    c = x.shape[1]
    ext.bn_eval(x.data_ptr(), out.data_ptr(),
                bn.weight.detach().float().contiguous().data_ptr(),
                bn.bias.detach().float().contiguous().data_ptr(),
                bn.running_mean.float().contiguous().data_ptr(),
                bn.running_var.float().contiguous().data_ptr(),
                x.numel(), c, hw, float(bn.eps), int(nhwc), int(relu),
                _dt(x), _stream())
    return out


_DRIFT_CHUNK = 1 << 16
_DRIFT_META: Dict = {}


class _L1DriftHipFn(torch.autograd.Function):

    @staticmethod
    def forward(ctx, meta, n_params, *tensors):
        ext = _ext_or_raise("drift")
        ptrs, chunks, sizes, total = meta
        partials = torch.empty(chunks.shape[0], device=tensors[0].device,
                               dtype=torch.float32)
        ext.drift_fwd(ptrs.data_ptr(), chunks.data_ptr(), partials.data_ptr(),
                      chunks.shape[0], _stream())
        ctx.meta = meta
        ctx.n_params = n_params
        ctx.shapes = [t.shape for t in tensors[:n_params]]
        return partials.sum()

    @staticmethod
    def backward(ctx, grad_out):
        ext = _ext_or_raise("drift")
        ptrs, chunks, sizes, total = ctx.meta
        flat = torch.empty(total, device=grad_out.device, dtype=torch.float32)
        g = grad_out.to(torch.float32).contiguous()
        ext.drift_bwd(ptrs.data_ptr(), chunks.data_ptr(), g.data_ptr(),
                      flat.data_ptr(), chunks.shape[0], _stream())
        views = [v.view(s) for v, s in zip(flat.split(sizes), ctx.shapes)]
        return (None, None, *views, *([None] * ctx.n_params))


def _drift_meta(pairs):
    key = tuple((p.data_ptr(), a.data_ptr(), p.numel()) for p, a in pairs)
    meta = _DRIFT_META.get(key)
    if meta is not None:
        return meta
    dev = pairs[0][0].device
    ptr_rows, chunk_rows, sizes = [], [], []
    flat_off = 0
    for i, (p, a) in enumerate(pairs):
        ptr_rows.append((p.data_ptr(), a.data_ptr()))
        n = p.numel()
        sizes.append(n)
        off = 0
        while off < n:
            ln = min(_DRIFT_CHUNK, n - off)
            chunk_rows.append((i, off, ln, flat_off + off))
            off += ln
        flat_off += n
    ptrs = torch.tensor(ptr_rows, dtype=torch.int64, device=dev)
    chunks = torch.tensor(chunk_rows, dtype=torch.int32, device=dev)
    meta = (ptrs, chunks, sizes, flat_off)
    _DRIFT_META[key] = meta
    return meta


def l1_drift(pairs) -> torch.Tensor:
    pairs = [(p, a.detach()) for p, a in pairs]
    if (pairs and pairs[0][0].is_cuda and extension_available()
            and all(p.dtype == torch.float32 and p.is_contiguous()
                    and a.dtype == torch.float32 and a.is_contiguous()
                    and p.numel() == a.numel() for p, a in pairs)):
        meta = _drift_meta(pairs)
        params = [p for p, _ in pairs]
        anchors = [a for _, a in pairs]
        return _L1DriftHipFn.apply(meta, len(params), *params, *anchors)
    return ref.l1_drift_fused(pairs)


class _BnTrain2dFn(torch.autograd.Function):

    @staticmethod
    def forward(ctx, x, gamma, beta, running_mean, running_var, momentum, eps,
                nbt, relu):
        ext = _ext_or_raise("bn_train")
        c = x.shape[1]
        m = x.numel() // c
        y = torch.empty_like(x)
        smean = torch.empty(c, device=x.device, dtype=torch.float32)
        sinv = torch.empty(c, device=x.device, dtype=torch.float32)
        nslab = ext.bn_train_nslab(m, c)
        part = torch.empty(2, nslab, c, device=x.device, dtype=torch.float32)
        has_rs = running_mean is not None
        ext.bn_train_fwd(
            x.data_ptr(), y.data_ptr(),
            gamma.detach().contiguous().data_ptr(),
            beta.detach().contiguous().data_ptr(),
            running_mean.data_ptr() if has_rs else 0,
            running_var.data_ptr() if has_rs else 0,
            smean.data_ptr(), sinv.data_ptr(),
            part[0].data_ptr(), part[1].data_ptr(),
            nbt.data_ptr() if nbt is not None else 0, m, c,
            float(momentum), float(eps), float(m) / float(m - 1),
            int(relu), _dt(x), _stream())
        ctx.save_for_backward(x, gamma, beta, smean, sinv)
        ctx.relu = bool(relu)
        return y

    @staticmethod
    def backward(ctx, dy):
        x, gamma, beta, smean, sinv = ctx.saved_tensors
        if x.dim() == 4:
            if not dy.is_contiguous(memory_format=torch.channels_last):
                dy = dy.contiguous(memory_format=torch.channels_last)
        elif not dy.is_contiguous():
            dy = dy.contiguous()
        if dy.dtype != x.dtype:
            dy = dy.to(x.dtype)
        ext = _ext_or_raise("bn_train")
        c = x.shape[1]
        m = x.numel() // c
        dx = torch.empty_like(x)
        dgamma = torch.empty(c, device=x.device, dtype=torch.float32)
        dbeta = torch.empty(c, device=x.device, dtype=torch.float32)
        nslab = ext.bn_train_nslab(m, c)
        part = torch.empty(2, nslab, c, device=x.device, dtype=torch.float32)
        ext.bn_train_bwd(x.data_ptr(), dy.data_ptr(), dx.data_ptr(),
                         gamma.detach().contiguous().data_ptr(),
                         beta.detach().contiguous().data_ptr(),
                         smean.data_ptr(), sinv.data_ptr(),
                         dgamma.data_ptr(), dbeta.data_ptr(),
                         part[0].data_ptr(), part[1].data_ptr(),
                         m, c, int(ctx.relu), _dt(x), _stream())
        return dx, dgamma, dbeta, None, None, None, None, None, None


def bn_train_2d(x: torch.Tensor, bn,
                relu: bool = False) -> Optional[torch.Tensor]:
    if os.environ.get("FLREID_NO_FUSED_BN", "0") == "1":
        return None
    if (not x.is_cuda or x.dtype not in (torch.float32, torch.bfloat16)
            or bn.weight is None or bn.bias is None):
        return None
    if x.dim() == 4:
        if not x.is_contiguous(memory_format=torch.channels_last):
            return None
    elif x.dim() == 2:
        if not x.is_contiguous():
            return None
    else:
        return None
    c = x.shape[1]
    m = x.numel() // c
    if c % 64 != 0 or m < 2 or m > 16384:
        return None
    if bn.momentum is None:
        return None
    if not extension_available():
        return None
    nbt = None
    if bn.track_running_stats and bn.running_mean is not None:
        nbt = bn.num_batches_tracked
        rm, rv = bn.running_mean, bn.running_var
    else:
        rm = rv = None
    return _BnTrain2dFn.apply(x, bn.weight, bn.bias, rm, rv,
                              bn.momentum, bn.eps, nbt, relu)


def _cl(t: torch.Tensor) -> torch.Tensor:
    return t if t.is_contiguous(memory_format=torch.channels_last) \
        else t.contiguous(memory_format=torch.channels_last)


def compose_theta_bf16(ext, gw: torch.Tensor, atten: Optional[torch.Tensor],
                       aw: Optional[torch.Tensor]) -> torch.Tensor:
    gw_d = gw.detach()
    if gw_d.dim() == 4:
        assert gw_d.is_contiguous(memory_format=torch.channels_last)
        inner, L = gw_d.shape[1], gw_d.shape[-1]
    else:
        assert gw_d.is_contiguous()
        inner = 1
        L = atten.numel() if atten is not None else 1
    if atten is not None:
        assert atten.numel() == L
    out = torch.empty_like(gw_d, dtype=torch.bfloat16)
    ext.compose2(gw_d.data_ptr(),
                 atten.detach().float().contiguous().data_ptr() if atten is not None else 0,
                 aw.detach().data_ptr() if aw is not None else 0,
                 out.data_ptr(), gw_d.numel(), L, inner, _dt(gw_d), _BF16,
                 _stream())
    return out


class _AdaptiveLinear1x1Fn(torch.autograd.Function):

    @staticmethod
    def forward(ctx, x, gw2d, atten, aw2d, bias):
        ext = _ext_or_raise("compose2")
        x_bf = x.detach().to(torch.bfloat16).contiguous()
        theta = compose_theta_bf16(ext, gw2d, atten, aw2d)
        y = x_bf @ theta.t()
        if bias is not None:
            y = y + bias.detach().to(torch.bfloat16)
        ctx.save_for_backward(x_bf, theta)
        ctx.x_dtype = x.dtype
        ctx.has_bias = bias is not None
        return y

    @staticmethod
    def backward(ctx, grad_out):
        x_bf, theta = ctx.saved_tensors
        g = grad_out.to(torch.bfloat16)
        dx = (g @ theta).to(ctx.x_dtype)
        d_aw = (g.t() @ x_bf).to(torch.float32)
        d_bias = grad_out.sum(0).to(torch.float32) if ctx.has_bias else None
        return dx, None, None, d_aw, d_bias


def adaptive_linear_1x1(x2d: torch.Tensor, gw2d: torch.Tensor,
                        atten: Optional[torch.Tensor],
                        aw2d: Optional[torch.Tensor],
                        bias: Optional[torch.Tensor]) -> Optional[torch.Tensor]:
    if (not x2d.is_cuda or not extension_available()
            or os.environ.get("FLREID_NO_FUSED_1X1", "0") == "1"):
        return None
    if gw2d.requires_grad or (atten is not None and atten.requires_grad):
        return None
    if x2d.dtype != torch.bfloat16 and not torch.is_autocast_enabled():
        return None
    if gw2d.dtype != torch.float32 or (aw2d is not None
                                       and aw2d.dtype != torch.float32):
        return None
    return _AdaptiveLinear1x1Fn.apply(x2d, gw2d, atten, aw2d, bias)


def conv_theta_tile(ext, w: torch.Tensor, atten: Optional[torch.Tensor],
                    aw: Optional[torch.Tensor], mode: int) -> torch.Tensor:
    w_d = w.detach()
    assert w_d.is_contiguous(memory_format=torch.channels_last)
    k, c = w_d.shape[0], w_d.shape[1]
    out = torch.empty(c * 9 * k, device=w.device, dtype=torch.bfloat16)
    ext.conv3x3_tile(
        w_d.data_ptr(),
        atten.detach().float().contiguous().data_ptr() if atten is not None else 0,
        aw.detach().data_ptr() if aw is not None else 0,
        out.data_ptr(), c, k, _dt(w_d), mode, _stream())
    return out


def conv_theta_flipt(ext, theta: torch.Tensor) -> torch.Tensor:
    k, c = theta.shape[0], theta.shape[1]
    flat = conv_theta_tile(ext, theta, None, None, mode=2)
    return flat.view(c, 3, 3, k).permute(0, 3, 1, 2)


def _conv_impl() -> str:
    return os.environ.get("FLREID_CONV_IMPL", "auto")


class _Conv3x3Fn(torch.autograd.Function):

    @staticmethod
    def forward(ctx, x, weight, atten, aw):
        ext = _ext_or_raise("conv3x3_img_fwd")
        x_bf = _cl(x.detach().to(torch.bfloat16))
        n, c, h, w = x_bf.shape
        k = weight.shape[0]
        hand = _conv_impl() == "hand"
        if hand:
            theta = compose_theta_bf16(ext, weight, atten, aw)
            y = torch.empty(n, k, h, w, device=x.device, dtype=torch.bfloat16,
                            memory_format=torch.channels_last)
            ext.conv3x3_img_fwd_ldsw(x_bf.data_ptr(), theta.data_ptr(),
                                     y.data_ptr(), n, h, w, c, k, _stream())
        else:
            theta = compose_theta_bf16(ext, weight, atten, aw)
            y = torch.nn.functional.conv2d(x_bf, theta, padding=1)
        ctx.save_for_backward(x_bf, weight, atten, aw,
                              None if hand else theta)
        ctx.x_dtype = x.dtype
        ctx.w_dtype = weight.dtype
        return y

    @staticmethod
    def backward(ctx, dy):
        ext = _ext_or_raise("conv3x3_img_fwd")
        x_bf, weight, atten, aw, theta = ctx.saved_tensors
        n, c, h, w = x_bf.shape
        k = weight.shape[0]
        hand = _conv_impl() == "hand"
        dy_bf = _cl(dy.to(torch.bfloat16))
        dx = None
        if ctx.needs_input_grad[0]:
            if hand:
                wt_tile = conv_theta_tile(ext, weight, atten, aw, mode=1)
                dx = torch.empty(n, c, h, w, device=dy.device,
                                 dtype=torch.bfloat16,
                                 memory_format=torch.channels_last)
                ext.conv3x3_img_fwd(dy_bf.data_ptr(), wt_tile.data_ptr(),
                                    dx.data_ptr(), n, h, w, k, c, _stream())
            else:
                if theta is None:
                    theta = compose_theta_bf16(ext, weight, atten, aw)
                if _conv_impl() == "lib":
                    dx = torch.nn.grad.conv2d_input((n, c, h, w), theta,
                                                    dy_bf, padding=1)
                else:
                    dx = torch.nn.functional.conv2d(
                        dy_bf, conv_theta_flipt(ext, theta), padding=1)
            if ctx.x_dtype != torch.bfloat16:
                dx = dx.to(ctx.x_dtype)
        d_weight = d_aw = None
        if ctx.needs_input_grad[1] or ctx.needs_input_grad[3]:
            if hand:
                m_rows = n * h * w
                dyt = torch.empty(k * m_rows + 256, device=dy.device,
                                  dtype=torch.bfloat16)
                xt = torch.empty(c * m_rows + 256, device=dy.device,
                                 dtype=torch.bfloat16)
                if m_rows % 64:
                    dyt[-128:].zero_()
                ext.transpose_bf16(dy_bf.data_ptr(), dyt.data_ptr() + 256,
                                   m_rows, k, _stream())
                ext.transpose_bf16(x_bf.data_ptr(), xt.data_ptr() + 256,
                                   m_rows, c, _stream())
                part = torch.empty(2, k * 9 * c, device=dy.device,
                                   dtype=torch.float32)
                ext.conv3x3_wgrad(dyt.data_ptr() + 256, xt.data_ptr() + 256,
                                  part.data_ptr(), n, h, w, c, k, _stream())
                dw = (part[0] + part[1]).view(k, 3, 3, c).permute(0, 3, 1, 2)
            else:
                dw = torch.nn.grad.conv2d_weight(
                    x_bf, (k, c, 3, 3), dy_bf, padding=1).to(torch.float32)
            if ctx.needs_input_grad[3]:
                d_aw = dw
            else:
                d_weight = dw if ctx.w_dtype == torch.float32 else dw.to(ctx.w_dtype)
        return dx, d_weight, None, d_aw


def conv3x3_try(x: torch.Tensor, weight: torch.Tensor,
                atten: Optional[torch.Tensor] = None,
                aw: Optional[torch.Tensor] = None) -> Optional[torch.Tensor]:
    if not x.is_cuda or x.dim() != 4 or not extension_available():
        return None
    if os.environ.get("FLREID_NO_FUSED_CONV", "0") == "1":
        return None
    n, c, h, w = x.shape
    k = weight.shape[0]
    hw = h * w
    if hw > 128 or hw % 16 or h + 2 > 18 or w + 2 > 10:
        return None
    if c % 32 or k % 32:
        return None
    if x.dtype != torch.bfloat16 and not torch.is_autocast_enabled():
        return None
    if weight.requires_grad and (aw is not None or atten is not None):
        return None
    if atten is not None and atten.requires_grad:
        return None
    if weight.dim() != 4 or not weight.is_contiguous(memory_format=torch.channels_last):
        return None
    if aw is not None and not aw.is_contiguous(memory_format=torch.channels_last):
        return None
    return _Conv3x3Fn.apply(x, weight, atten, aw)


def conv3x3_fwd_nhwc(x: torch.Tensor, weight: torch.Tensor) -> torch.Tensor:
    n, c, h, w = x.shape
    k = weight.shape[0]
    if c % 32 != 0 or k % 16 != 0:
        return torch.nn.functional.conv2d(x, weight.to(x.dtype), padding=1)
    ext = _ext_or_raise("conv3x3_fwd")
    assert x.is_contiguous(memory_format=torch.channels_last)
    wcl = weight.detach()
    if not wcl.is_contiguous(memory_format=torch.channels_last):
        wcl = wcl.contiguous(memory_format=torch.channels_last)
    out = torch.empty(n, k, h, w, device=x.device,
                      dtype=torch.bfloat16).to(memory_format=torch.channels_last)
    ext.conv3x3_fwd(x.data_ptr(), wcl.float().data_ptr(), out.data_ptr(),
                    n, h, w, c, k, _stream())
    return out
```

flreid_amd/ops/build.py:

```python

from __future__ import annotations

import os
import subprocess
import sys
import sysconfig

CSRC = os.path.join(os.path.dirname(os.path.abspath(__file__)), "csrc")
OUT = os.path.join(os.path.dirname(os.path.abspath(__file__)), "_flreid_hip.so")

SOURCES = ["module.cpp", "elementwise.hip", "distance.hip", "window_attn.hip", "triplet.hip", "adaptive_gemm.hip", "conv3x3.hip", "conv3x3_img.hip", "conv3x3_img_ldsw.hip", "bn_train.hip", "drift.hip", "kd.hip", "patch_merge.hip", "decomposed.hip"]


def _pybind11_includes():
    import pybind11
    return [pybind11.get_include()]


def needs_rebuild() -> bool:
    if not os.path.exists(OUT):
        return True
    out_mtime = os.path.getmtime(OUT)
    for f in os.listdir(CSRC):
        if os.path.getmtime(os.path.join(CSRC, f)) > out_mtime:
            return True
    return False


def build(force: bool = False, arch: str = "gfx950", verbose: bool = True,
          debug: bool = False, asan: bool = False) -> str:
    if not force and not needs_rebuild():
        if verbose:
            print(f"[flreid build] up to date: {OUT}")
        return OUT
    hipcc = os.environ.get("HIPCC", "/opt/rocm/bin/hipcc")
    includes = [sysconfig.get_paths()["include"]] + _pybind11_includes()
    debug = debug or os.environ.get("FLREID_BUILD_DEBUG", "0") == "1"
    asan = asan or os.environ.get("FLREID_BUILD_ASAN", "0") == "1"
    opt = ["-g", "-O1"] if (debug or asan) else ["-O3"]
    extra = []
    if asan:
        extra = ["-fsanitize=address", "-shared-libsan",
                 "-Xarch_device", "-fno-sanitize=all"]
    cmd = [
        hipcc, f"--offload-arch={arch}", *opt, *extra, "-std=c++17", "-fPIC",
        "-shared", "-fvisibility=hidden",
        *[f"-I{p}" for p in includes],
        *[os.path.join(CSRC, s) for s in SOURCES],
        "-o", OUT,
    ]
    if verbose:
        print("[flreid build]", " ".join(cmd))
    subprocess.run(cmd, check=True)
    return OUT


if __name__ == "__main__":
    build(force=any(f in sys.argv for f in ("--force", "--debug", "--asan")),
          debug="--debug" in sys.argv, asan="--asan" in sys.argv)
```

flreid_amd/ops/csrc/adaptive_gemm.hip:

```cpp

#include "common.h"

namespace flreid {

using bf16x8 = __attribute__((ext_vector_type(8))) __bf16;
using f32x4 = __attribute__((ext_vector_type(4))) float;

constexpr int AG_BM = 64;
constexpr int AG_BN = 32;
constexpr int AG_BK = 32;
constexpr int AG_PAD = 2;

struct Prefetch {
  ushort4 xr[4];
  float4 gr[2], ar[2];
};

__global__ __launch_bounds__(128) void adaptive_linear_fwd_kernel(
    const __hip_bfloat16* __restrict__ X, const float* __restrict__ GW,
    const float* __restrict__ AW, const float* __restrict__ ATTEN,
    const float* __restrict__ BIAS, __hip_bfloat16* __restrict__ OUT,
    int M, int N, int K) {
  __shared__ __hip_bfloat16 lx[2][AG_BM][AG_BK + AG_PAD];
  __shared__ __hip_bfloat16 lth[2][AG_BN][AG_BK + AG_PAD];

  const int m0 = blockIdx.x * AG_BM;
  const int n0 = blockIdx.y * AG_BN;
  const int tid = threadIdx.x;
  const int lane = tid & 63;
  const int wave = tid >> 6;
  const int fn = wave * 16 + (lane & 15);

  const int lc4 = (tid & 7) * 4;
  const int lr0 = tid >> 3;
  const bool edge = (m0 + AG_BM > M) || (n0 + AG_BN > N);

  f32x4 acc[4] = {{}, {}, {}, {}};

  auto load_tile = [&](int k0, Prefetch& p) {
    if (!edge) {
#pragma unroll
      for (int i = 0; i < 4; ++i) {
        p.xr[i] = *(const ushort4*)(X + (int64_t)(m0 + lr0 + 16 * i) * K + k0 + lc4);
      }
#pragma unroll
      for (int i = 0; i < 2; ++i) {
        const int64_t base = (int64_t)(n0 + lr0 + 16 * i) * K + k0 + lc4;
        p.gr[i] = *(const float4*)(GW + base);
        p.ar[i] = AW ? *(const float4*)(AW + base) : float4{0.f, 0.f, 0.f, 0.f};
      }
    } else {
#pragma unroll
      for (int i = 0; i < 4; ++i) {
        const int mr = m0 + lr0 + 16 * i;
        ushort4 v = {0, 0, 0, 0};
        if (mr < M) {
          v = *(const ushort4*)(X + (int64_t)mr * K + k0 + lc4);
        }
        p.xr[i] = v;
      }
#pragma unroll
      for (int i = 0; i < 2; ++i) {
        const int nr = n0 + lr0 + 16 * i;
        float4 g = {0.f, 0.f, 0.f, 0.f}, a = {0.f, 0.f, 0.f, 0.f};
        if (nr < N) {
          const int64_t base = (int64_t)nr * K + k0 + lc4;
          g = *(const float4*)(GW + base);
          if (AW) a = *(const float4*)(AW + base);
        }
        p.gr[i] = g;
        p.ar[i] = a;
      }
    }
  };

  auto store_tile = [&](int k0, const Prefetch& p, int buf) {
#pragma unroll
    for (int i = 0; i < 4; ++i) {
      __hip_bfloat16* dst = &lx[buf][lr0 + 16 * i][lc4];
      dst[0] = *(const __hip_bfloat16*)&p.xr[i].x;
      dst[1] = *(const __hip_bfloat16*)&p.xr[i].y;
      dst[2] = *(const __hip_bfloat16*)&p.xr[i].z;
      dst[3] = *(const __hip_bfloat16*)&p.xr[i].w;
    }
    float at[4] = {1.f, 1.f, 1.f, 1.f};
    if (ATTEN) {
      at[0] = ATTEN[k0 + lc4 + 0];
      at[1] = ATTEN[k0 + lc4 + 1];
      at[2] = ATTEN[k0 + lc4 + 2];
      at[3] = ATTEN[k0 + lc4 + 3];
    }
#pragma unroll
    for (int i = 0; i < 2; ++i) {
      __hip_bfloat16* dst = &lth[buf][lr0 + 16 * i][lc4];
      dst[0] = __float2bfloat16(fmaf(at[0], p.gr[i].x, p.ar[i].x));
      dst[1] = __float2bfloat16(fmaf(at[1], p.gr[i].y, p.ar[i].y));
      dst[2] = __float2bfloat16(fmaf(at[2], p.gr[i].z, p.ar[i].z));
      dst[3] = __float2bfloat16(fmaf(at[3], p.gr[i].w, p.ar[i].w));
    }
  };

  const int NT = K / AG_BK;
  Prefetch cur_p, next_p;
  load_tile(0, cur_p);
  store_tile(0, cur_p, 0);
  __syncthreads();

  int buf = 0;
  const int kg = (lane >> 4) * 4;
  for (int t = 0; t < NT; ++t) {
    if (t + 1 < NT) {
      load_tile((t + 1) * AG_BK, next_p);
    }

    bf16x8 bfrag;
#pragma unroll
    for (int e = 0; e < 8; ++e) {
      const int kk = e < 4 ? kg + e : 16 + kg + e - 4;
      bfrag[e] = *reinterpret_cast<const __bf16*>(&lth[buf][fn][kk]);
    }
#pragma unroll
    for (int mf = 0; mf < 4; ++mf) {
      bf16x8 afrag;
#pragma unroll
      for (int e = 0; e < 8; ++e) {
        const int kk = e < 4 ? kg + e : 16 + kg + e - 4;
        afrag[e] = *reinterpret_cast<const __bf16*>(
            &lx[buf][mf * 16 + (lane & 15)][kk]);
      }
      acc[mf] = __builtin_amdgcn_mfma_f32_16x16x32_bf16(afrag, bfrag, acc[mf],
                                                        0, 0, 0);
    }

    if (t + 1 < NT) {
      store_tile((t + 1) * AG_BK, next_p, buf ^ 1);
    }
    __syncthreads();
    buf ^= 1;
  }

  const int nc = n0 + fn;
  if (nc >= N) return;
  const float bias_v = BIAS ? BIAS[nc] : 0.0f;
#pragma unroll
  for (int mf = 0; mf < 4; ++mf) {
#pragma unroll
    for (int reg = 0; reg < 4; ++reg) {
      const int mr = m0 + mf * 16 + (lane >> 4) * 4 + reg;
      if (mr < M) {
        OUT[(int64_t)mr * N + nc] = __float2bfloat16(acc[mf][reg] + bias_v);
      }
    }
  }
}

extern "C" void flreid_adaptive_linear_fwd(
    const void* X, const float* GW, const float* AW, const float* ATTEN,
    const float* BIAS, void* OUT, int M, int N, int K, int split_layout,
    hipStream_t stream) {
  (void)split_layout;
  if (K % AG_BK != 0) {
    throw std::runtime_error("adaptive_linear_fwd: K must be a multiple of 32");
  }
  dim3 grid((M + AG_BM - 1) / AG_BM, (N + AG_BN - 1) / AG_BN);
  dim3 block(128);
  hipLaunchKernelGGL((adaptive_linear_fwd_kernel), grid, block, 0, stream,
                     (const __hip_bfloat16*)X, GW, AW, ATTEN, BIAS,
                     (__hip_bfloat16*)OUT, M, N, K);
  HIP_CHECK(hipGetLastError());
}

}
```

flreid_amd/ops/csrc/module.cpp:

```cpp

#include <pybind11/pybind11.h>

#include <cstdint>

#include <hip/hip_runtime.h>

namespace flreid {
extern "C" void flreid_l2norm_rows(const void*, void*, int64_t, int64_t, int,
                                   float, hipStream_t);
extern "C" void flreid_ce_smooth(const void*, const int64_t*, float*, void*,
                                 int64_t, int64_t, int, float, hipStream_t);
extern "C" void flreid_compose(const void*, const float*, const void*, void*,
                               int64_t, int64_t, int, hipStream_t);
extern "C" void flreid_importance(float*, const void*, int64_t, int, int,
                                  float, hipStream_t);
extern "C" void flreid_pairwise(const float*, const float*, const float*,
                                const float*, float*, int64_t, int64_t,
                                int64_t, int, hipStream_t);
extern "C" void flreid_rowsq(const float*, float*, int64_t, int64_t,
                             hipStream_t);
extern "C" void flreid_window_attn_fwd(const void*, const void*, const void*,
                                       const float*, const float*, void*,
                                       int64_t, int, int, int, int, float,
                                       int, hipStream_t);
extern "C" void flreid_window_attn_bwd(const void*, const void*, const void*,
                                       const float*, const float*,
                                       const void*, void*, void*, void*,
                                       float*, int64_t, int, int, int, int,
                                       float, int, hipStream_t);
extern "C" void flreid_triplet_fwd(const float*, const float*, const int64_t*,
                                   float*, int*, int*, int, int, float,
                                   hipStream_t);
extern "C" void flreid_triplet_bwd(const float*, const float*, const int*,
                                   const int*, float*, int, int, float,
                                   hipStream_t);
extern "C" void flreid_adaptive_linear_fwd(const void*, const float*,
                                           const float*, const float*,
                                           const float*, void*, int, int,
                                           int, int, hipStream_t);
extern "C" void flreid_bn_eval(const void*, void*, const float*, const float*,
                               const float*, const float*, int64_t, int,
                               int64_t, float, int, int, int, hipStream_t);
extern "C" void flreid_conv3x3_fwd(const void*, const float*, void*, int, int,
                                   int, int, int, hipStream_t);
extern "C" int flreid_bn_train_nslab(int64_t, int);
extern "C" void flreid_bn_train_fwd(const void*, void*, const float*,
                                    const float*, float*, float*, float*,
                                    float*, float*, float*,
                                    unsigned long long*, int64_t, int, float,
                                    float, float, int, int, hipStream_t);
extern "C" void flreid_bn_train_bwd(const void*, const void*, void*,
                                    const float*, const float*, const float*,
                                    const float*, float*, float*, float*,
                                    float*, int64_t, int, int, int,
                                    hipStream_t);
extern "C" void flreid_compose2(const void*, const float*, const void*,
                                void*, int64_t, int64_t, int64_t, int, int,
                                hipStream_t);
extern "C" void flreid_conv3x3_img_fwd(const void*, const void*, void*, int,
                                       int, int, int, int, hipStream_t);
extern "C" void flreid_transpose_bf16(const void*, void*, int64_t, int64_t,
                                      hipStream_t);
extern "C" void flreid_conv3x3_tile(const void*, const float*, const void*,
                                    void*, int, int, int, int, hipStream_t);
extern "C" void flreid_conv3x3_img_fwd_ldsw(const void*, const void*, void*,
                                            int, int, int, int, int,
                                            hipStream_t);
extern "C" void flreid_conv3x3_wgrad(const void*, const void*, float*, int,
                                     int, int, int, int, hipStream_t);
extern "C" void flreid_patch_merge_ln_fwd(const void*, const float*,
                                          const float*, void*, float*,
                                          float*, int64_t, int, int, int,
                                          float, int, hipStream_t);
extern "C" void flreid_patch_merge_ln_bwd(const void*, const float*,
                                          const void*, const float*,
                                          const float*, void*, float*,
                                          float*, int64_t, int, int, int,
                                          int, hipStream_t);
extern "C" void flreid_kd_fwd(const float*, const float*, float*, float*,
                              int64_t, int64_t, float, hipStream_t);
extern "C" void flreid_icarl_distill(const float*, const int64_t*,
                                     const float*, float*, float*, int64_t,
                                     int64_t, int64_t, hipStream_t);
extern "C" void flreid_drift_fwd(const int64_t*, const int*, float*, int,
                                 hipStream_t);
extern "C" void flreid_drift_bwd(const int64_t*, const int*, const float*,
                                 float*, int, hipStream_t);
extern "C" void flreid_decomposed_plan(int64_t, int64_t, int64_t, int,
                                       int64_t*, int64_t*);
extern "C" void flreid_decomposed_fwd(const float*, const float*,
                                      const float*, const float*,
                                      const float*, void*, int64_t, int64_t,
                                      int64_t, int64_t, int, int, float,
                                      float, int, hipStream_t);
extern "C" void flreid_decomposed_bwd(const void*, int, const float*,
                                      const float*, const float*,
                                      const float*, float*, float*, float*,
                                      int64_t, int64_t, int64_t, int64_t, int,
                                      int, float, float, int, int, int,
                                      hipStream_t);
}

namespace py = pybind11;

static hipStream_t as_stream(uintptr_t s) {
  return reinterpret_cast<hipStream_t>(s);
}

PYBIND11_MODULE(_flreid_hip, m) {
  m.doc() = "flreid MI355X (gfx950) kernels";

  m.def("l2norm_rows",
        [](uintptr_t x, uintptr_t y, int64_t rows, int64_t cols, int dtype,
           float eps, uintptr_t stream) {
          flreid::flreid_l2norm_rows((const void*)x, (void*)y, rows, cols,
                                     dtype, eps, as_stream(stream));
        });

  m.def("ce_smooth",
        [](uintptr_t score, uintptr_t target, uintptr_t row_loss,
           uintptr_t grad, int64_t B, int64_t C, int dtype, float eps,
           uintptr_t stream) {
          flreid::flreid_ce_smooth((const void*)score, (const int64_t*)target,
                                   (float*)row_loss, (void*)grad, B, C, dtype,
                                   eps, as_stream(stream));
        });

  m.def("compose",
        [](uintptr_t gw, uintptr_t atten, uintptr_t aw, uintptr_t out,
           int64_t numel, int64_t L, int dtype, uintptr_t stream) {
          flreid::flreid_compose((const void*)gw, (const float*)atten,
                                 (const void*)aw, (void*)out, numel, L, dtype,
                                 as_stream(stream));
        });

  m.def("importance",
        [](uintptr_t F, uintptr_t g, int64_t numel, int dtype, bool sq,
           float scale, uintptr_t stream) {
          flreid::flreid_importance((float*)F, (const void*)g, numel, dtype,
                                    sq ? 1 : 0, scale, as_stream(stream));
        });

  m.def("pairwise",
        [](uintptr_t A, uintptr_t B, uintptr_t aa, uintptr_t bb, uintptr_t out,
           int64_t M, int64_t N, int64_t D, int mode, uintptr_t stream) {
          flreid::flreid_pairwise((const float*)A, (const float*)B,
                                  (const float*)aa, (const float*)bb,
                                  (float*)out, M, N, D, mode,
                                  as_stream(stream));
        });

  m.def("rowsq", [](uintptr_t x, uintptr_t out, int64_t rows, int64_t cols,
                    uintptr_t stream) {
    flreid::flreid_rowsq((const float*)x, (float*)out, rows, cols,
                         as_stream(stream));
  });

  m.def("window_attn_fwd",
        [](uintptr_t q, uintptr_t k, uintptr_t v, uintptr_t bias,
           uintptr_t mask, uintptr_t out, int64_t BW, int H, int N, int D,
           int nW, float scale, int dtype, uintptr_t stream) {
          flreid::flreid_window_attn_fwd(
              (const void*)q, (const void*)k, (const void*)v,
              (const float*)bias, (const float*)mask, (void*)out, BW, H, N, D,
              nW, scale, dtype, as_stream(stream));
        });

  m.def("window_attn_bwd",
        [](uintptr_t q, uintptr_t k, uintptr_t v, uintptr_t bias,
           uintptr_t mask, uintptr_t dout, uintptr_t dq, uintptr_t dk,
           uintptr_t dv, uintptr_t ds, int64_t BW, int H, int N, int D,
           int nW, float scale, int dtype, uintptr_t stream) {
          flreid::flreid_window_attn_bwd(
              (const void*)q, (const void*)k, (const void*)v,
              (const float*)bias, (const float*)mask, (const void*)dout,
              (void*)dq, (void*)dk, (void*)dv, (float*)ds, BW, H, N, D, nW,
              scale, dtype, as_stream(stream));
        });

  m.def("triplet_fwd",
        [](uintptr_t F, uintptr_t norms, uintptr_t labels, uintptr_t row_loss,
           uintptr_t p_idx, uintptr_t n_idx, int N, int D, float margin,
           uintptr_t stream) {
          flreid::flreid_triplet_fwd((const float*)F, (const float*)norms,
                                     (const int64_t*)labels, (float*)row_loss,
                                     (int*)p_idx, (int*)n_idx, N, D, margin,
                                     as_stream(stream));
        });

  m.def("adaptive_linear_fwd",
        [](uintptr_t X, uintptr_t GW, uintptr_t AW, uintptr_t ATTEN,
           uintptr_t BIAS, uintptr_t OUT, int M, int N, int K,
           int split_layout, uintptr_t stream) {
          flreid::flreid_adaptive_linear_fwd(
              (const void*)X, (const float*)GW, (const float*)AW,
              (const float*)ATTEN, (const float*)BIAS, (void*)OUT, M, N, K,
              split_layout, as_stream(stream));
        });

  m.def("bn_eval",
        [](uintptr_t x, uintptr_t y, uintptr_t gamma, uintptr_t beta,
           uintptr_t mean, uintptr_t var, int64_t numel, int C, int64_t HW,
           float eps, int nhwc, int relu, int dtype, uintptr_t stream) {
          flreid::flreid_bn_eval((const void*)x, (void*)y,
                                 (const float*)gamma, (const float*)beta,
                                 (const float*)mean, (const float*)var, numel,
                                 C, HW, eps, nhwc, relu, dtype,
                                 as_stream(stream));
        });

  m.def("conv3x3_fwd",
        [](uintptr_t x, uintptr_t w, uintptr_t y, int NB, int H, int Wd,
           int C, int K, uintptr_t stream) {
          flreid::flreid_conv3x3_fwd((const void*)x, (const float*)w,
                                     (void*)y, NB, H, Wd, C, K,
                                     as_stream(stream));
        });

  m.def("bn_train_nslab", [](int64_t M, int C) {
    return flreid::flreid_bn_train_nslab(M, C);
  });

  m.def("bn_train_fwd",
        [](uintptr_t x, uintptr_t y, uintptr_t gamma, uintptr_t beta,
           uintptr_t rmean, uintptr_t rvar, uintptr_t smean, uintptr_t sinv,
           uintptr_t part_a, uintptr_t part_b, uintptr_t nbt, int64_t M,
           int C, float momentum, float eps, float unbiased, int relu,
           int dtype, uintptr_t stream) {
          flreid::flreid_bn_train_fwd((const void*)x, (void*)y,
                                      (const float*)gamma, (const float*)beta,
                                      (float*)rmean, (float*)rvar,
                                      (float*)smean, (float*)sinv,
                                      (float*)part_a, (float*)part_b,
                                      (unsigned long long*)nbt, M, C,
                                      momentum, eps, unbiased, relu, dtype,
                                      as_stream(stream));
        });

  m.def("bn_train_bwd",
        [](uintptr_t x, uintptr_t dy, uintptr_t dx, uintptr_t gamma,
           uintptr_t beta, uintptr_t smean, uintptr_t sinv, uintptr_t dgamma,
           uintptr_t dbeta, uintptr_t part_a, uintptr_t part_b, int64_t M,
           int C, int relu, int dtype, uintptr_t stream) {
          flreid::flreid_bn_train_bwd((const void*)x, (const void*)dy,
                                      (void*)dx, (const float*)gamma,
                                      (const float*)beta, (const float*)smean,
                                      (const float*)sinv, (float*)dgamma,
                                      (float*)dbeta, (float*)part_a,
                                      (float*)part_b, M, C, relu, dtype,
                                      as_stream(stream));
        });

  m.def("compose2",
        [](uintptr_t gw, uintptr_t atten, uintptr_t aw, uintptr_t out,
           int64_t numel, int64_t L, int64_t inner, int in_dtype,
           int out_dtype, uintptr_t stream) {
          flreid::flreid_compose2((const void*)gw, (const float*)atten,
                                  (const void*)aw, (void*)out, numel, L,
                                  inner, in_dtype, out_dtype,
                                  as_stream(stream));
        });

  m.def("conv3x3_img_fwd",
        [](uintptr_t x, uintptr_t w, uintptr_t y, int NB, int H, int Wd,
           int C, int K, uintptr_t stream) {
          flreid::flreid_conv3x3_img_fwd((const void*)x, (const void*)w,
                                         (void*)y, NB, H, Wd, C, K,
                                         as_stream(stream));
        });

  m.def("transpose_bf16",
        [](uintptr_t in, uintptr_t out, int64_t M, int64_t N,
           uintptr_t stream) {
          flreid::flreid_transpose_bf16((const void*)in, (void*)out, M, N,
                                        as_stream(stream));
        });

  m.def("conv3x3_img_fwd_ldsw",
        [](uintptr_t x, uintptr_t w, uintptr_t y, int NB, int H, int Wd,
           int C, int K, uintptr_t stream) {
          flreid::flreid_conv3x3_img_fwd_ldsw((const void*)x, (const void*)w,
                                              (void*)y, NB, H, Wd, C, K,
                                              as_stream(stream));
        });

  m.def("conv3x3_tile",
        [](uintptr_t gw, uintptr_t atten, uintptr_t aw, uintptr_t out,
           int C, int K, int in_dtype, int mode, uintptr_t stream) {
          flreid::flreid_conv3x3_tile((const void*)gw, (const float*)atten,
                                      (const void*)aw, (void*)out, C, K,
                                      in_dtype, mode, as_stream(stream));
        });

  m.def("conv3x3_wgrad",
        [](uintptr_t dy, uintptr_t x, uintptr_t dw, int NB, int H, int Wd,
           int C, int K, uintptr_t stream) {
          flreid::flreid_conv3x3_wgrad((const void*)dy, (const void*)x,
                                       (float*)dw, NB, H, Wd, C, K,
                                       as_stream(stream));
        });

  m.def("patch_merge_ln_fwd",
        [](uintptr_t x, uintptr_t gamma, uintptr_t beta, uintptr_t y,
           uintptr_t mean, uintptr_t rstd, int64_t rows, int C, int H,
           int W, float eps, int dtype, uintptr_t stream) {
          flreid::flreid_patch_merge_ln_fwd(
              (const void*)x, (const float*)gamma, (const float*)beta,
              (void*)y, (float*)mean, (float*)rstd, rows, C, H, W, eps,
              dtype, as_stream(stream));
        });

  m.def("patch_merge_ln_bwd",
        [](uintptr_t x, uintptr_t gamma, uintptr_t dy, uintptr_t mean,
           uintptr_t rstd, uintptr_t dx, uintptr_t dg, uintptr_t db,
           int64_t rows, int C, int H, int W, int dtype, uintptr_t stream) {
          flreid::flreid_patch_merge_ln_bwd(
              (const void*)x, (const float*)gamma, (const void*)dy,
              (const float*)mean, (const float*)rstd, (void*)dx, (float*)dg,
              (float*)db, rows, C, H, W, dtype, as_stream(stream));
        });

  m.def("kd_fwd",
        [](uintptr_t zs, uintptr_t zt, uintptr_t row_loss, uintptr_t grad,
           int64_t B, int64_t C, float temperature, uintptr_t stream) {
          flreid::flreid_kd_fwd((const float*)zs, (const float*)zt,
                                (float*)row_loss, (float*)grad, B, C,
                                temperature, as_stream(stream));
        });

  m.def("icarl_distill",
        [](uintptr_t score, uintptr_t target, uintptr_t prev,
           uintptr_t row_loss, uintptr_t grad, int64_t B, int64_t C,
           int64_t P, uintptr_t stream) {
          flreid::flreid_icarl_distill((const float*)score,
                                       (const int64_t*)target,
                                       (const float*)prev, (float*)row_loss,
                                       (float*)grad, B, C, P,
                                       as_stream(stream));
        });

  m.def("drift_fwd",
        [](uintptr_t ptrs, uintptr_t chunks, uintptr_t partials, int n_chunks,
           uintptr_t stream) {
          flreid::flreid_drift_fwd((const int64_t*)ptrs, (const int*)chunks,
                                   (float*)partials, n_chunks,
                                   as_stream(stream));
        });

  m.def("drift_bwd",
        [](uintptr_t ptrs, uintptr_t chunks, uintptr_t gscale,
           uintptr_t flat_grad, int n_chunks, uintptr_t stream) {
          flreid::flreid_drift_bwd((const int64_t*)ptrs, (const int*)chunks,
                                   (const float*)gscale, (float*)flat_grad,
                                   n_chunks, as_stream(stream));
        });

  m.def("triplet_bwd",
        [](uintptr_t F, uintptr_t row_loss, uintptr_t p_idx, uintptr_t n_idx,
           uintptr_t grad, int N, int D, float coeff, uintptr_t stream) {
          flreid::flreid_triplet_bwd((const float*)F, (const float*)row_loss,
                                     (const int*)p_idx, (const int*)n_idx,
                                     (float*)grad, N, D, coeff,
                                     as_stream(stream));
        });

  m.def("decomposed_plan",
        [](int64_t rows, int64_t C, int64_t S, int channels_last) {
          int64_t tpr = 0, blocks = 0;
          flreid::flreid_decomposed_plan(rows, C, S, channels_last, &tpr,
                                         &blocks);
          return py::make_tuple(tpr, blocks);
        });

  m.def("decomposed_fwd",
        [](uintptr_t sw, uintptr_t mask, uintptr_t aw, uintptr_t aw_kb,
           uintptr_t atten, uintptr_t out, int64_t rows, int64_t C, int64_t S,
           int64_t KB, int channels_last, int train, float lambda_l1,
           float lambda_mask, int out_dtype, uintptr_t stream) {
          flreid::flreid_decomposed_fwd(
              (const float*)sw, (const float*)mask, (const float*)aw,
              (const float*)aw_kb, (const float*)atten, (void*)out, rows, C,
              S, KB, channels_last, train, lambda_l1, lambda_mask, out_dtype,
              as_stream(stream));
        });

  m.def("decomposed_bwd",
        [](uintptr_t g, int g_dtype, uintptr_t sw, uintptr_t mask,
           uintptr_t aw, uintptr_t aw_kb, uintptr_t d_aw,
           uintptr_t dmask_part, uintptr_t datten_part, int64_t rows,
           int64_t C, int64_t S, int64_t KB, int channels_last, int train,
           float lambda_l1, float lambda_mask, int need_aw, int need_mask,
           int need_atten, uintptr_t stream) {
          flreid::flreid_decomposed_bwd(
              (const void*)g, g_dtype, (const float*)sw, (const float*)mask,
              (const float*)aw, (const float*)aw_kb, (float*)d_aw,
              (float*)dmask_part, (float*)datten_part, rows, C, S, KB,
              channels_last, train, lambda_l1, lambda_mask, need_aw,
              need_mask, need_atten, as_stream(stream));
        });
}
```

flreid_amd/ops/reference.py:

```python

from __future__ import annotations

from typing import Dict, Iterable, Optional, Tuple

import torch
import torch.nn.functional as F



def pairwise_sqeuclidean(a: torch.Tensor, b: torch.Tensor) -> torch.Tensor:
    m, n = a.size(0), b.size(0)
    aa = a.pow(2).sum(dim=1, keepdim=True).expand(m, n)
    bb = b.pow(2).sum(dim=1, keepdim=True).expand(n, m).t()
    return torch.addmm(aa + bb, a, b.t(), beta=1, alpha=-2)


def pairwise_cosine_distance(a: torch.Tensor, b: torch.Tensor) -> torch.Tensor:
    a = F.normalize(a, p=2, dim=1)
    b = F.normalize(b, p=2, dim=1)
    return 1.0 - a @ b.t()


def kl_distance(a: torch.Tensor, b: torch.Tensor) -> torch.Tensor:
    return F.kl_div(F.log_softmax(a, dim=-1), F.softmax(b, dim=-1), reduction="sum")


def l2_normalize(x: torch.Tensor, dim: int = 1, eps: float = 1e-12) -> torch.Tensor:
    return F.normalize(x, p=2, dim=dim, eps=eps)



def ce_label_smooth(score: torch.Tensor, target: torch.Tensor,
                    epsilon: float = 0.1) -> torch.Tensor:
    num_classes = score.size(1)
    log_probs = F.log_softmax(score, dim=1)
    with torch.no_grad():
        tgt = torch.zeros_like(log_probs).scatter_(1, target.view(-1, 1), 1.0)
        tgt = (1.0 - epsilon) * tgt + epsilon / num_classes
    return (-tgt * log_probs).mean(0).sum()


def _softmax_weights(dist: torch.Tensor, mask: torch.Tensor) -> torch.Tensor:
    max_v = torch.max(dist * mask, dim=1, keepdim=True)[0]
    diff = dist - max_v
    z = torch.sum(torch.exp(diff) * mask, dim=1, keepdim=True) + 1e-6
    return torch.exp(diff) * mask / z


def triplet_loss(feature: torch.Tensor, target: torch.Tensor,
                 margin: Optional[float] = 0.3, norm_feat: bool = False,
                 hard_mining: bool = True) -> torch.Tensor:
    if norm_feat:
        dist = pairwise_cosine_distance(feature, feature)
    else:
        dist = pairwise_sqeuclidean(feature, feature)

    n = dist.size(0)
    is_pos = target.view(n, 1).eq(target.view(1, n)).to(dist.dtype)
    is_neg = 1.0 - is_pos

    if hard_mining:
        dist_ap = torch.max(dist * is_pos, dim=1)[0]
        dist_an = torch.min(dist * is_neg + is_pos * 1e9, dim=1)[0]
    else:
        w_ap = _softmax_weights(dist * is_pos, is_pos)
        w_an = _softmax_weights(-dist * is_neg, is_neg)
        dist_ap = torch.sum(dist * is_pos * w_ap, dim=1)
        dist_an = torch.sum(dist * is_neg * w_an, dim=1)

    y = torch.ones_like(dist_an)
    if margin is not None and margin > 0:
        return F.margin_ranking_loss(dist_an, dist_ap, y, margin=margin)
    loss = F.soft_margin_loss(dist_an - dist_ap, y)
    if loss == float("inf"):
        loss = F.margin_ranking_loss(dist_an, dist_ap, y, margin=0.3)
    return loss


def icarl_distill_loss(score: torch.Tensor, target: torch.Tensor,
                       prev_logits: torch.Tensor) -> torch.Tensor:
    from flreid_amd.tools.utils import get_one_hot

    p = prev_logits.shape[1]
    clf = F.binary_cross_entropy_with_logits(
        score.float(), get_one_hot(target, score.shape[1]))
    distill = F.binary_cross_entropy_with_logits(
        score[:, :p].float(), torch.sigmoid(prev_logits.float()))
    return clf + distill


def kd_loss(logits_student: torch.Tensor, logits_teacher: torch.Tensor,
            temperature: float = 4.0) -> torch.Tensor:
    t = temperature
    p_s = F.log_softmax(logits_student / t, dim=1)
    p_t = F.softmax(logits_teacher / t, dim=1)
    return F.kl_div(p_s, p_t, reduction="sum") * (t * t) / logits_student.size(0)



def importance_update(importance: Dict[str, torch.Tensor],
                      grads: Dict[str, torch.Tensor],
                      mode: str = "sq", scale: float = 1.0) -> None:
    for n, g in grads.items():
        if g is None:
            continue
        if mode == "sq":
            importance[n] += (g.detach().float() ** 2) * scale
        elif mode == "abs":
            importance[n] += g.detach().float().abs() * scale
        else:
            raise ValueError(mode)


def quadratic_penalty(params: Dict[str, torch.Tensor],
                      anchors: Dict[str, torch.Tensor],
                      importance: Optional[Dict[str, torch.Tensor]] = None,
                      ) -> torch.Tensor:
    total = None
    for n, p in params.items():
        if n not in anchors:
            continue
        d = (p - anchors[n]) ** 2
        if importance is not None:
            d = importance[n] * d
        s = d.sum()
        total = s if total is None else total + s
    if total is None:
        total = torch.zeros((), device=next(iter(params.values())).device)
    return total


def l1_drift(pairs: Iterable[Tuple[torch.Tensor, torch.Tensor]]) -> torch.Tensor:
    total = None
    for p, p0 in pairs:
        s = (p - p0).abs().sum()
        total = s if total is None else total + s
    return total


class _L1DriftFusedFn(torch.autograd.Function):

    @staticmethod
    def forward(ctx, n_params, *tensors):
        params = list(tensors[:n_params])
        anchors = list(tensors[n_params:])
        diffs = torch._foreach_sub(params, anchors)
        ctx.n_params = n_params
        ctx.save_for_backward(*diffs)
        norms = torch._foreach_norm(diffs, 1)
        return torch.stack(norms).sum()

    @staticmethod
    def backward(ctx, grad_out):
        diffs = list(ctx.saved_tensors)
        signs = torch._foreach_sign(diffs)
        torch._foreach_mul_(signs, grad_out)
        return (None, *signs, *([None] * ctx.n_params))


def l1_drift_fused(pairs) -> torch.Tensor:
    pairs = list(pairs)
    params = [p for p, _ in pairs]
    anchors = [p0.detach() for _, p0 in pairs]
    return _L1DriftFusedFn.apply(len(params), *params, *anchors)



def adaptive_compose(global_weight: torch.Tensor, atten: torch.Tensor,
                     adaptive_weight: torch.Tensor) -> torch.Tensor:
    return atten * global_weight + adaptive_weight



def l1_hard_threshold(weights: torch.Tensor, threshold: float) -> torch.Tensor:
    return weights * torch.greater(weights.abs(), threshold).to(weights.dtype)


def decomposed_compose(sw: torch.Tensor, mask: torch.Tensor, aw: torch.Tensor,
                       aw_kb: torch.Tensor, atten: torch.Tensor,
                       lambda_l1: float, lambda_mask: float,
                       training: bool) -> torch.Tensor:
    if training:
        aw = l1_hard_threshold(aw, lambda_l1)
        mask = l1_hard_threshold(mask, lambda_mask)
    kb = (atten * aw_kb).sum(dim=-1)
    return mask.view((-1,) + (1,) * (sw.dim() - 1)) * sw + aw + kb



@torch.no_grad()
def cmc_map(query_features: torch.Tensor, query_labels: torch.Tensor,
            gallery_features: torch.Tensor, gallery_labels: torch.Tensor,
            query_camera_labels: Optional[torch.Tensor] = None,
            gallery_camera_labels: Optional[torch.Tensor] = None,
            ) -> Tuple[torch.Tensor, float]:
    sims = query_features.float() @ gallery_features.float().t()
    return cmc_map_from_sims(sims, query_labels, gallery_labels,
                             query_camera_labels, gallery_camera_labels)


@torch.no_grad()
def cmc_map_from_sims(sims: torch.Tensor, query_labels: torch.Tensor,
                      gallery_labels: torch.Tensor,
                      query_camera_labels: Optional[torch.Tensor] = None,
                      gallery_camera_labels: Optional[torch.Tensor] = None,
                      ) -> Tuple[torch.Tensor, float]:
    q, g = sims.shape
    device = sims.device
    ql = query_labels.to(device).view(q, 1)
    gl = gallery_labels.to(device).view(1, g)

    same_id = ql.eq(gl)
    if query_camera_labels is not None and gallery_camera_labels is not None:
        qc = query_camera_labels.to(device).view(q, 1)
        gc = gallery_camera_labels.to(device).view(1, g)
        same_cam = qc.eq(gc)
        junk = (gl.expand(q, g) == -1) | (same_id & same_cam)
        good = same_id & ~same_cam & (gl.expand(q, g) != -1)
    else:
        junk = torch.zeros_like(same_id)
        good = same_id

    order = torch.flip(torch.argsort(sims, dim=1, descending=False, stable=True),
                       dims=[1])
    good_sorted = good.gather(1, order)
    valid_sorted = (~junk).gather(1, order)

    rank_in_valid = valid_sorted.long().cumsum(dim=1) - 1
    hit = good_sorted & valid_sorted

    big = g + 1
    first_rank = torch.where(hit, rank_in_valid, torch.full_like(rank_in_valid, big))
    r0 = first_rank.min(dim=1)[0]
    has_good = r0 < big
    cmc = torch.zeros(g, dtype=torch.float64, device=device)
    if has_good.any():
        hist = torch.bincount(r0[has_good], minlength=g + 1)[:g].to(torch.float64)
        cmc = hist.cumsum(0)
    cmc = cmc / q

    hit_idx = hit.long().cumsum(dim=1) - 1
    r = rank_in_valid.to(torch.float64)
    i = hit_idx.to(torch.float64)
    precision = (i + 1.0) / (r + 1.0)
    old_precision = torch.where(r > 0, i / r.clamp(min=1), torch.ones_like(r))
    contrib = torch.where(hit, (precision + old_precision) * 0.5, torch.zeros_like(r))
    n_good = hit.sum(dim=1).to(torch.float64)
    ap = contrib.sum(dim=1) / n_good.clamp(min=1)
    ap = torch.where(has_good, ap, torch.zeros_like(ap))
    return cmc.cpu(), float(ap.sum().item() / q)



def window_attention(q: torch.Tensor, k: torch.Tensor, v: torch.Tensor,
                     bias: torch.Tensor, mask: Optional[torch.Tensor],
                     scale: float, dropout=None) -> torch.Tensor:
    bn, h, n, _d = q.shape
    attn = (q * scale) @ k.transpose(-2, -1) + bias.unsqueeze(0).to(q.dtype)
    if mask is not None:
        nw = mask.shape[0]
        attn = attn.view(bn // nw, nw, h, n, n) \
            + mask.unsqueeze(1).unsqueeze(0).to(attn.dtype)
        attn = attn.view(bn, h, n, n)
    attn = F.softmax(attn.float(), dim=-1).to(q.dtype)
    if dropout is not None:
        attn = dropout(attn)
    return attn @ v
```

Baseline: 4344 images/sec.

## Fuse adaptive-weight Adam step, L1 drift and bf16 theta composition into one kernel

Adds a multi-tensor HIP kernel that performs the Adam update for the adaptive weights together with the L1 drift-to-anchor gradient, the drift sum, and the recomputation of the composed bf16 weight (atten*gw+aw). The drift loss leaves the autograd graph, and the forward pass reads a precomputed 'live theta' buffer through a custom autograd function whose gradient is routed into the fused step. This removes separate compose, drift-loss forward/backward and per-parameter optimizer kernels from each head step. In exchange it adds a large amount of fragile plumbing (graph cache keys, pointer-keyed plans, bf16 gradients for fp32 params) that could change numerics slightly.

```diff
diff --git a/flreid_amd/methods/common.py b/flreid_amd/methods/common.py
--- a/flreid_amd/methods/common.py
+++ b/flreid_amd/methods/common.py
@@ -29,6 +29,152 @@
         if not zeroed:
             optimizer.state = collections.defaultdict(dict)
             return
+
+
+def fused_head_step_enabled() -> bool:
+    return os.environ.get("FLREID_FUSED_HEAD_STEP", "1") != "0"
+
+
+class FusedHeadStep:
+
+    def __init__(self, leaves, states, group, live: bool):
+        self.leaves = leaves
+        self.live = live
+        self.rows = self._rows(leaves, states)
+        self.theta = []
+        if live:
+            for r, leaf in zip(self.rows, leaves):
+                r["gw"] = leaf.global_weight.data
+                r["atten"] = leaf.global_weight_atten.data
+                r["theta"] = torch.empty_like(r["aw"], dtype=torch.bfloat16)
+                self.theta.append(r["theta"])
+        n = ops.head_step_partials(self.rows)
+        self.partials = torch.zeros(n + 1, dtype=torch.float64,
+                                    device=self.rows[0]["aw"].device)
+        self.key = self._key(leaves, self.rows, live)
+        self.begin_epoch(group)
+
+    @staticmethod
+    def _rows(leaves, states):
+        return [{"aw": l.adaptive_weight.data,
+                 "aw0": l.initial_adaptive_weight.data, "m": s["exp_avg"],
+                 "v": s["exp_avg_sq"], "step": s["step"]}
+                for l, s in zip(leaves, states)]
+
+    @staticmethod
+    def _key(leaves, rows, live):
+        return (live,) + tuple(
+            tuple(r[k].data_ptr() for k in ("aw", "aw0", "m", "v", "step"))
+            + (l.global_weight.data_ptr(), l.global_weight_atten.data_ptr())
+            for l, r in zip(leaves, rows))
+
+    def begin_epoch(self, group) -> None:
+        beta1, beta2 = group["betas"]
+        self.hyper = (float(group["lr"]), float(beta1), float(beta2),
+                      float(group["weight_decay"]), float(group["eps"]))
+        with torch.no_grad():
+            c = ops.l1_drift([(l.global_weight_atten.detach(),
+                               l.initial_global_weight_atten.detach())
+                              for l in self.leaves])
+            self.partials[-1:].copy_(c.to(torch.float64).reshape(1))
+
+    def live_theta(self):
+        import contextlib
+
+        from flreid_amd.models.adaptive import live_theta_scope
+        if not self.live:
+            return contextlib.nullcontext()
+        return live_theta_scope(self.leaves, self.theta)
+
+    @torch.no_grad()
+    def step(self, lam: float) -> None:
+        for r, leaf in zip(self.rows, self.leaves):
+            p, slot = leaf.adaptive_weight, leaf._live
+            dw = slot.grad if slot is not None else p.grad
+            r["dw"] = dw if dw is not None else torch.zeros_like(p)
+        ops.head_step(self.rows, self.partials, *self.hyper, lam)
+        for r, leaf in zip(self.rows, self.leaves):
+            r["dw"] = None
+            leaf.adaptive_weight.grad = None
+            if leaf._live is not None:
+                leaf._live.grad = None
+
+    def drift(self) -> torch.Tensor:
+        return self.partials.sum().to(torch.float32)
+
+    @classmethod
+    def plan(cls, model, optimizer, device, previous=None):
+        from flreid_amd.models.adaptive import (
+            AdaptiveConv2d,
+            AdaptiveLinear,
+            live_theta_enabled,
+        )
+        from flreid_amd.runtime.precision import bf16_enabled
+
+        if not (fused_head_step_enabled() and str(device).startswith("cuda")
+                and bf16_enabled() and ops.extension_available()):
+            return None
+        if type(optimizer) is not torch.optim.Adam \
+                or len(optimizer.param_groups) != 1:
+            return None
+        group = optimizer.param_groups[0]
+        if (not group.get("fused") or group.get("amsgrad")
+                or group.get("maximize") or group.get("differentiable")
+                or group.get("decoupled_weight_decay")
+                or torch.is_tensor(group["lr"])):
+            return None
+        in_group = {id(p) for p in group["params"]}
+        leaves = []
+        live = live_theta_enabled()
+        for _n, leaf in model.adaptive_module_leaves():
+            if type(leaf) not in (AdaptiveLinear, AdaptiveConv2d):
+                return None
+            p, a = leaf.adaptive_weight, leaf.initial_adaptive_weight
+            gw, atten = leaf.global_weight, leaf.global_weight_atten
+            if (gw.requires_grad or atten.requires_grad
+                    or not p.requires_grad or id(p) not in in_group
+                    or not p.is_cuda or p.dtype != torch.float32
+                    or a.dtype != torch.float32
+                    or not ops._same_layout(a, p)
+                    or atten.shape != leaf.initial_global_weight_atten.shape):
+                return None
+            try:
+                L, _inner = ops._head_step_geometry(p)
+            except ValueError:
+                return None
+            if (gw.dtype != torch.float32 or not ops._same_layout(gw, p)
+                    or atten.dtype != torch.float32
+                    or not atten.is_contiguous() or atten.numel() != L):
+                live = False
+            leaves.append(leaf)
+        if not leaves:
+            return None
+        states = []
+        for leaf in leaves:
+            p = leaf.adaptive_weight
+            st = optimizer.state[p]
+            if len(st) == 0:
+                st["step"] = torch.zeros((), dtype=torch.float32,
+                                         device=p.device)
+                st["exp_avg"] = torch.zeros_like(
+                    p, memory_format=torch.preserve_format)
+                st["exp_avg_sq"] = torch.zeros_like(
+                    p, memory_format=torch.preserve_format)
+            step = st.get("step")
+            if (not torch.is_tensor(step) or not step.is_cuda
+                    or step.dtype != torch.float32
+                    or not all(torch.is_tensor(st.get(k))
+                               and st[k].dtype == torch.float32
+                               and ops._same_layout(st[k], p)
+                               for k in ("exp_avg", "exp_avg_sq"))):
+                return None
+            states.append(st)
+        if previous is not None and previous.key == cls._key(
+                leaves, cls._rows(leaves, states), live):
+            previous.leaves = leaves
+            previous.begin_epoch(group)
+            return previous
+        return cls(leaves, states, group, live)
 
 
 class BaseReIDOperator(OperatorModule):
diff --git a/flreid_amd/methods/fedstil.py b/flreid_amd/methods/fedstil.py
--- a/flreid_amd/methods/fedstil.py
+++ b/flreid_amd/methods/fedstil.py
@@ -1,6 +1,7 @@
 
 from __future__ import annotations
 
+import contextlib
 import math
 from typing import Any, Dict, List, Optional
 
@@ -8,7 +9,11 @@
 from torch.utils.data import DataLoader
 
 from flreid_amd import ops
-from flreid_amd.methods.common import BaseReIDClient, BaseReIDOperator
+from flreid_amd.methods.common import (
+    BaseReIDClient,
+    BaseReIDOperator,
+    FusedHeadStep,
+)
 from flreid_amd.models.adaptive import (
     adaptive_leaves,
     convert_to_adaptive,
@@ -306,6 +311,16 @@
                    self.classes.index_select(0, idx_cpu))
 
 
+@contextlib.contextmanager
+def head_epoch(model, operator, capturable: bool = True):
+    operator.set_optimizer_parameters(model, capturable=capturable)
+    plan = FusedHeadStep.plan(model, operator.optimizer, model.device,
+                              previous=getattr(operator, "_fused_head", None))
+    operator._fused_head = plan
+    with plan.live_theta() if plan is not None else contextlib.nullcontext():
+        yield plan
+
+
 class Operator(BaseReIDOperator):
     def generate_proto_loader(self, model: Model, source_loader: DataLoader):
         device = model.device
@@ -370,17 +385,24 @@
     def _train_step(self, model: Model, data: torch.Tensor,
                     target: torch.Tensor):
         device = model.device
+        fused = getattr(self, "_fused_head", None)
         self.optimizer.zero_grad(set_to_none=True)
         with autocast(device):
             score, feature = model.head_forward(data)
             loss = 0.0
             for loss_func in self.criterion:
                 loss = loss + loss_func(score=score, feature=feature, target=target)
-            loss = loss + model.drift_loss() * model.lambda_l1
+            if fused is None:
+                loss = loss + model.drift_loss() * model.lambda_l1
         loss.backward()
+        if fused is not None:
+            fused.step(model.lambda_l1)
         self.optimizer.step()
+        loss = loss.detach()
+        if fused is not None:
+            loss = loss + fused.drift() * model.lambda_l1
         b_acc = (score.detach().argmax(dim=1) == target).sum()
-        return loss.detach(), b_acc
+        return loss, b_acc
 
     def _graphed_step(self, model: Model, batch_size: int):
         from flreid_amd.runtime.hipgraph import GraphedStep
@@ -388,7 +410,8 @@
         lr = self.optimizer.param_groups[0]["lr"]
         shapes = tuple(tuple(p.shape) for p in
                        self.optimizer.param_groups[0]["params"])
-        key = (batch_size, float(lr), shapes)
+        key = (batch_size, float(lr), shapes,
+               id(getattr(self, "_fused_head", None)))
         cache = getattr(self, "_train_graphs", None)
         if cache is None or cache[0] != key:
             gs = GraphedStep(lambda d, t: self._train_step(model, d, t))
@@ -403,7 +426,8 @@
         lr = float(self.optimizer.param_groups[0]["lr"])
         shapes = tuple(tuple(p.shape) for p in
                        self.optimizer.param_groups[0]["params"])
-        key = (tuple(loader.data.shape), batch, steps, lr, shapes)
+        key = (tuple(loader.data.shape), batch, steps, lr, shapes,
+               id(getattr(self, "_fused_head", None)))
         cache = getattr(self, "_epoch_graph_cache", None)
         if cache is None or cache[0] != key:
             eg = EpochGraph(lambda d, t: self._train_step(model, d, t),
@@ -424,59 +448,59 @@
             proto_loader, task_token = self.generate_proto_loader(model, dataloader)
 
         model.train()
-        self.set_optimizer_parameters(model, capturable=use_graph)
         batch_size = getattr(proto_loader, "batch_size", None)
-        _phase_head = phase("head_epoch"); _phase_head.__enter__()
-
-        use_epoch = (use_graph and epoch_graph_enabled()
-                     and isinstance(proto_loader, TensorBatches)
-                     and proto_loader.data.is_cuda
-                     and proto_loader._pids_dev is not None
-                     and proto_loader.data.shape[0] >= batch_size)
-        if use_epoch:
-            n = proto_loader.data.shape[0]
-            steps = n // batch_size
-            order = torch.randperm(n)
-            eg = self._epoch_graph(model, proto_loader)
-            idx_flat = order[:steps * batch_size].to(device, non_blocking=True)
-            loss_dev, acc_dev = eg.run(proto_loader.data,
-                                       proto_loader._pids_dev, idx_flat)
-            batch_cnt, data_cnt = steps, steps * batch_size
-            stop = (steps * batch_size
-                    if (proto_loader.drop_last or n % batch_size == 0) else n)
-            if stop > steps * batch_size:
-                tail = order[steps * batch_size:stop].to(device)
-                d = proto_loader.present(
-                    proto_loader.data.index_select(0, tail))
-                t = proto_loader._pids_dev.index_select(0, tail)
-                b_loss, b_acc = self._train_step(model, d, t)
-                loss_dev = loss_dev + b_loss
-                acc_dev = acc_dev + b_acc
-                batch_cnt += 1
-                data_cnt += tail.numel()
-        else:
-            gs = self._graphed_step(model, batch_size) if use_graph else None
-            warmups = 0
-
-            acc_dev = loss_dev = None
-            for data, person_id, _class_id in proto_loader:
-                data = data.to(device, non_blocking=True)
-                target = person_id.to(device, non_blocking=True)
-                if gs is not None and data.shape[0] == batch_size:
-                    if gs.ready:
-                        b_loss, b_acc = gs(data, target)
-                    elif warmups < 2:
-                        b_loss, b_acc = gs.warmup(data, target)
-                        warmups += 1
+        with contextlib.ExitStack() as scope:
+            scope.enter_context(phase("head_epoch"))
+            scope.enter_context(head_epoch(model, self, capturable=use_graph))
+
+            use_epoch = (use_graph and epoch_graph_enabled()
+                         and isinstance(proto_loader, TensorBatches)
+                         and proto_loader.data.is_cuda
+                         and proto_loader._pids_dev is not None
+                         and proto_loader.data.shape[0] >= batch_size)
+            if use_epoch:
+                n = proto_loader.data.shape[0]
+                steps = n // batch_size
+                order = torch.randperm(n)
+                eg = self._epoch_graph(model, proto_loader)
+                idx_flat = order[:steps * batch_size].to(device, non_blocking=True)
+                loss_dev, acc_dev = eg.run(proto_loader.data,
+                                           proto_loader._pids_dev, idx_flat)
+                batch_cnt, data_cnt = steps, steps * batch_size
+                stop = (steps * batch_size
+                        if (proto_loader.drop_last or n % batch_size == 0) else n)
+                if stop > steps * batch_size:
+                    tail = order[steps * batch_size:stop].to(device)
+                    d = proto_loader.present(
+                        proto_loader.data.index_select(0, tail))
+                    t = proto_loader._pids_dev.index_select(0, tail)
+                    b_loss, b_acc = self._train_step(model, d, t)
+                    loss_dev = loss_dev + b_loss
+                    acc_dev = acc_dev + b_acc
+                    batch_cnt += 1
+                    data_cnt += tail.numel()
+            else:
+                gs = self._graphed_step(model, batch_size) if use_graph else None
+                warmups = 0
+
+                acc_dev = loss_dev = None
+                for data, person_id, _class_id in proto_loader:
+                    data = data.to(device, non_blocking=True)
+                    target = person_id.to(device, non_blocking=True)
+                    if gs is not None and data.shape[0] == batch_size:
+                        if gs.ready:
+                            b_loss, b_acc = gs(data, target)
+                        elif warmups < 2:
+                            b_loss, b_acc = gs.warmup(data, target)
+                            warmups += 1
+                        else:
+                            b_loss, b_acc = gs.capture(data, target)
                     else:
-                        b_loss, b_acc = gs.capture(data, target)
-                else:
-                    b_loss, b_acc = self._train_step(model, data, target)
-                acc_dev = b_acc.clone() if acc_dev is None else acc_dev + b_acc
-                loss_dev = b_loss.clone() if loss_dev is None else loss_dev + b_loss
-                data_cnt += len(data)
-                batch_cnt += 1
-        _phase_head.__exit__(None, None, None)
+                        b_loss, b_acc = self._train_step(model, data, target)
+                    acc_dev = b_acc.clone() if acc_dev is None else acc_dev + b_acc
+                    loss_dev = b_loss.clone() if loss_dev is None else loss_dev + b_loss
+                    data_cnt += len(data)
+                    batch_cnt += 1
         if acc_dev is not None:
             train_acc = float(acc_dev)
             train_loss = float(loss_dev)
diff --git a/flreid_amd/models/adaptive.py b/flreid_amd/models/adaptive.py
--- a/flreid_amd/models/adaptive.py
+++ b/flreid_amd/models/adaptive.py
@@ -1,6 +1,7 @@
 
 from __future__ import annotations
 
+import contextlib
 import os
 from typing import Optional, Tuple
 
@@ -12,7 +13,56 @@
 from flreid_amd import ops
 
 
+def live_theta_enabled() -> bool:
+    return os.environ.get("FLREID_LIVE_THETA", "1") != "0"
+
+
+class _LiveThetaFn(torch.autograd.Function):
+
+    @staticmethod
+    def forward(ctx, aw, live):
+        ctx.live = live
+        return live.theta.detach()
+
+    @staticmethod
+    def backward(ctx, g):
+        live = ctx.live
+        if g.dtype != torch.bfloat16:
+            g = g.to(torch.bfloat16)
+        if not ops._same_layout(g, live.theta):
+            g = torch.empty_like(live.theta).copy_(g)
+        live.grad = g if live.grad is None else live.grad + g
+        return None, None
+
+
+class LiveTheta:
+
+    def __init__(self, theta: torch.Tensor):
+        self.theta = theta
+        self.grad: Optional[torch.Tensor] = None
+
+    def __call__(self, adaptive_weight: torch.Tensor) -> torch.Tensor:
+        return _LiveThetaFn.apply(adaptive_weight, self)
+
+
+@contextlib.contextmanager
+def live_theta_scope(leaves, buffers):
+    ext = ops._ext_or_raise("compose2")
+    try:
+        for leaf, buf in zip(leaves, buffers):
+            ops.compose_theta_bf16(ext, leaf.global_weight,
+                                   leaf.global_weight_atten,
+                                   leaf.adaptive_weight, out=buf)
+            leaf._live = LiveTheta(buf)
+        yield
+    finally:
+        for leaf in leaves:
+            leaf._live = None
+
+
 class AdaptiveBase(nn.Module):
+
+    _live: Optional[LiveTheta] = None
 
     def __init__(self, global_weight: torch.Tensor,
                  global_weight_atten: Optional[torch.Tensor] = None,
@@ -77,6 +127,13 @@
 
 class AdaptiveLinear(AdaptiveBase):
     def forward(self, data: torch.Tensor) -> torch.Tensor:
+        if self._live is not None:
+            theta = self._live(self.adaptive_weight)
+            k2 = os.environ.get("FLREID_CLASSIFIER_GEMM", "k2") != "lib"
+            y = ops.theta_linear(data, theta, self.adaptive_bias, k2=k2) \
+                if data.dim() == 2 else None
+            return y if y is not None else F.linear(data, theta,
+                                                    self.adaptive_bias)
         if data.dim() == 2:
             return ops.adaptive_linear(data, self.global_weight,
                                        self.global_weight_atten,
@@ -99,7 +156,28 @@
         self.stride = stride
         self.padding = padding
 
-    def forward(self, data: torch.Tensor) -> torch.Tensor:
+    def _forward_live(self, data: torch.Tensor) -> torch.Tensor:
+        theta = self._live(self.adaptive_weight)
+        k = theta.shape
+        if (k[2] == 3 and k[3] == 3 and _is_one(self.stride)
+                and _is_one(self.padding) and self.adaptive_bias is None):
+            y = ops.conv3x3_try(data, theta)
+            if y is not None:
+                return y
+        if (k[2] == 1 and k[3] == 1 and _is_one(self.stride)
+                and _is_zero(self.padding)
+                and os.environ.get("FLREID_NO_FUSED_1X1", "0") != "1"):
+            b, c, h, w = data.shape
+            xv = data.permute(0, 2, 3, 1).reshape(-1, c)
+            y = ops.theta_linear(xv, theta.view(k[0], c), self.adaptive_bias)
+            if y is not None:
+                return y.view(b, h, w, -1).permute(0, 3, 1, 2)
+        return F.conv2d(data, theta, self.adaptive_bias,
+                        stride=self.stride, padding=self.padding)
+
+    def forward(self, data: torch.Tensor) -> torch.Tensor:
+        if self._live is not None and self.global_weight.dim() == 4:
+            return self._forward_live(data)
         gw = self.global_weight
         if (data.is_cuda and gw.dim() == 4 and gw.shape[2] == 3
                 and gw.shape[3] == 3 and _is_one(self.stride)
diff --git a/flreid_amd/ops/__init__.py b/flreid_amd/ops/__init__.py
--- a/flreid_amd/ops/__init__.py
+++ b/flreid_amd/ops/__init__.py
@@ -824,9 +824,12 @@
 
 
 def compose_theta_bf16(ext, gw: torch.Tensor, atten: Optional[torch.Tensor],
-                       aw: Optional[torch.Tensor]) -> torch.Tensor:
+                       aw: Optional[torch.Tensor],
+                       out: Optional[torch.Tensor] = None) -> torch.Tensor:
     gw_d = gw.detach()
-    if gw_d.dim() == 4:
+    if gw_d.dim() == 4 and gw_d.is_contiguous():
+        inner, L = 1, gw_d.shape[-1]
+    elif gw_d.dim() == 4:
         assert gw_d.is_contiguous(memory_format=torch.channels_last)
         inner, L = gw_d.shape[1], gw_d.shape[-1]
     else:
@@ -835,7 +838,10 @@
         L = atten.numel() if atten is not None else 1
     if atten is not None:
         assert atten.numel() == L
-    out = torch.empty_like(gw_d, dtype=torch.bfloat16)
+    if out is None:
+        out = torch.empty_like(gw_d, dtype=torch.bfloat16)
+    elif out.dtype != torch.bfloat16 or not _same_layout(out, gw_d):
+        raise ValueError("compose_theta_bf16: out must be bf16 in gw's layout")
     ext.compose2(gw_d.data_ptr(),
                  atten.detach().float().contiguous().data_ptr() if atten is not None else 0,
                  aw.detach().data_ptr() if aw is not None else 0,
@@ -867,6 +873,54 @@
         d_aw = (g.t() @ x_bf).to(torch.float32)
         d_bias = grad_out.sum(0).to(torch.float32) if ctx.has_bias else None
         return dx, None, None, d_aw, d_bias
+
+
+class _ThetaLinearFn(torch.autograd.Function):
+
+    @staticmethod
+    def forward(ctx, x, theta, bias, k2):
+        x_bf = x.detach().to(torch.bfloat16).contiguous()
+        th = theta.detach()
+        if k2:
+            ext = _ext_or_raise("theta_linear_fwd")
+            m, k = x_bf.shape
+            n = th.shape[0]
+            y = torch.empty(m, n, device=x.device, dtype=torch.bfloat16)
+            ext.theta_linear_fwd(
+                x_bf.data_ptr(), th.data_ptr(),
+                bias.detach().contiguous().float().data_ptr()
+                if bias is not None else 0,
+                y.data_ptr(), m, n, k, _stream())
+        else:
+            y = x_bf @ th.t()
+            if bias is not None:
+                y = y + bias.detach().to(torch.bfloat16)
+        ctx.save_for_backward(x_bf, th)
+        ctx.x_dtype = x.dtype
+        ctx.has_bias = bias is not None
+        return y
+
+    @staticmethod
+    def backward(ctx, grad_out):
+        x_bf, th = ctx.saved_tensors
+        g = grad_out.to(torch.bfloat16)
+        dx = (g @ th).to(ctx.x_dtype) if ctx.needs_input_grad[0] else None
+        d_theta = g.t() @ x_bf
+        d_bias = grad_out.sum(0).to(torch.float32) if ctx.has_bias else None
+        return dx, d_theta, d_bias, None
+
+
+def theta_linear(x2d: torch.Tensor, theta2d: torch.Tensor,
+                 bias: Optional[torch.Tensor],
+                 k2: bool = False) -> Optional[torch.Tensor]:
+    if (not x2d.is_cuda or x2d.dim() != 2 or not extension_available()
+            or theta2d.dtype != torch.bfloat16
+            or not theta2d.is_contiguous()):
+        return None
+    if x2d.dtype != torch.bfloat16 and not torch.is_autocast_enabled():
+        return None
+    return _ThetaLinearFn.apply(x2d, theta2d, bias,
+                                bool(k2) and theta2d.shape[1] % 32 == 0)
 
 
 def adaptive_linear_1x1(x2d: torch.Tensor, gw2d: torch.Tensor,
@@ -919,14 +973,16 @@
         n, c, h, w = x_bf.shape
         k = weight.shape[0]
         hand = _conv_impl() == "hand"
+        if weight.dtype == torch.bfloat16 and atten is None and aw is None:
+            theta = weight.detach()
+        else:
+            theta = compose_theta_bf16(ext, weight, atten, aw)
         if hand:
-            theta = compose_theta_bf16(ext, weight, atten, aw)
             y = torch.empty(n, k, h, w, device=x.device, dtype=torch.bfloat16,
                             memory_format=torch.channels_last)
             ext.conv3x3_img_fwd_ldsw(x_bf.data_ptr(), theta.data_ptr(),
                                      y.data_ptr(), n, h, w, c, k, _stream())
         else:
-            theta = compose_theta_bf16(ext, weight, atten, aw)
             y = torch.nn.functional.conv2d(x_bf, theta, padding=1)
         ctx.save_for_backward(x_bf, weight, atten, aw,
                               None if hand else theta)
@@ -983,11 +1039,14 @@
                 dw = (part[0] + part[1]).view(k, 3, 3, c).permute(0, 3, 1, 2)
             else:
                 dw = torch.nn.grad.conv2d_weight(
-                    x_bf, (k, c, 3, 3), dy_bf, padding=1).to(torch.float32)
+                    x_bf, (k, c, 3, 3), dy_bf, padding=1)
+            want = torch.float32 if ctx.needs_input_grad[3] else ctx.w_dtype
+            if dw.dtype != want:
+                dw = dw.to(want)
             if ctx.needs_input_grad[3]:
                 d_aw = dw
             else:
-                d_weight = dw if ctx.w_dtype == torch.float32 else dw.to(ctx.w_dtype)
+                d_weight = dw
         return dx, d_weight, None, d_aw
 
 
@@ -1033,3 +1092,142 @@
     ext.conv3x3_fwd(x.data_ptr(), wcl.float().data_ptr(), out.data_ptr(),
                     n, h, w, c, k, _stream())
     return out
+
+
+
+HEAD_STEP_CHUNK = 1 << 14
+_HS_GRAD_BF16, _HS_VEC, _HS_THETA, _HS_ATTEN_VEC = 1, 2, 4, 8
+
+
+def _same_layout(t: torch.Tensor, like: torch.Tensor) -> bool:
+    return t.shape == like.shape and all(
+        a == b for a, b, n in zip(t.stride(), like.stride(), like.shape)
+        if n > 1)
+
+
+def head_step_partials(rows) -> int:
+    return sum(-(-r["aw"].numel() // HEAD_STEP_CHUNK) for r in rows)
+
+
+def _head_step_geometry(aw: torch.Tensor):
+    if aw.dim() < 1 or aw.numel() == 0:
+        raise ValueError("head_step: empty adaptive weight")
+    if aw.is_contiguous():
+        return aw.shape[-1], 1
+    if aw.dim() == 4 and aw.is_contiguous(memory_format=torch.channels_last):
+        return aw.shape[-1], aw.shape[1]
+    raise ValueError("head_step: adaptive weight is neither contiguous nor "
+                     f"channels-last dense (strides {aw.stride()})")
+
+
+def _head_step_row(r: Dict, partial0: int):
+    aw = r["aw"]
+    if not aw.is_cuda or aw.dtype != torch.float32:
+        raise TypeError("head_step: aw must be a CUDA fp32 tensor")
+    L, inner = _head_step_geometry(aw)
+    for k in ("aw0", "m", "v", "dw"):
+        t = r.get(k)
+        if t is None:
+            raise ValueError(f"head_step: missing '{k}' (null pointer)")
+        if not t.is_cuda or t.device != aw.device:
+            raise TypeError(f"head_step: '{k}' is not on aw's device")
+        if t.numel() != aw.numel() or not _same_layout(t, aw):
+            raise ValueError(
+                f"head_step: '{k}' {tuple(t.shape)}/{t.stride()} does not "
+                f"match aw's layout {tuple(aw.shape)}/{aw.stride()}")
+        if k == "dw":
+            if t.dtype not in (torch.float32, torch.bfloat16):
+                raise TypeError("head_step: dw must be fp32 or bf16")
+        elif t.dtype != torch.float32:
+            raise TypeError(f"head_step: '{k}' must be fp32")
+    step = r.get("step")
+    if (step is None or not step.is_cuda or step.dtype != torch.float32
+            or step.numel() != 1):
+        raise TypeError("head_step: step must be a CUDA fp32 scalar tensor")
+    dw = r["dw"]
+    flags = _HS_GRAD_BF16 if dw.dtype == torch.bfloat16 else 0
+    gw, atten, theta = r.get("gw"), r.get("atten"), r.get("theta")
+    has_theta = theta is not None
+    if has_theta:
+        if gw is None or atten is None:
+            raise ValueError("head_step: theta needs gw and atten "
+                             "(null pointer)")
+        if (gw.dtype != torch.float32 or gw.device != aw.device
+                or not _same_layout(gw, aw)):
+            raise ValueError("head_step: gw does not match aw's layout")
+        if (theta.dtype != torch.bfloat16 or theta.device != aw.device
+                or not _same_layout(theta, aw)):
+            raise ValueError("head_step: theta must be bf16 in aw's layout")
+        if (atten.dtype != torch.float32 or atten.device != aw.device
+                or not atten.is_contiguous() or atten.numel() != L):
+            raise ValueError("head_step: atten must be a contiguous fp32 "
+                             f"vector of the last weight dim ({L})")
+        flags |= _HS_THETA
+    galign = 8 if dw.dtype == torch.bfloat16 else 16
+    vec = (all(r[k].data_ptr() % 16 == 0 for k in ("aw", "aw0", "m", "v"))
+           and dw.data_ptr() % galign == 0)
+    if vec and has_theta:
+        vec = gw.data_ptr() % 16 == 0 and theta.data_ptr() % 8 == 0
+        if vec and inner == 1 and L > 1 and L % 4 == 0 \
+                and atten.data_ptr() % 16 == 0:
+            flags |= _HS_ATTEN_VEC
+        elif not (L == 1 or inner % 4 == 0):
+            vec = False
+    if vec:
+        flags |= _HS_VEC
+    return [aw.data_ptr(), r["aw0"].data_ptr(), dw.data_ptr(),
+            gw.data_ptr() if has_theta else 0,
+            atten.data_ptr() if has_theta else 0,
+            r["m"].data_ptr(), r["v"].data_ptr(),
+            theta.data_ptr() if has_theta else 0, step.data_ptr(),
+            aw.numel(), L, inner, flags, partial0]
+
+
+def _head_step_cpu(rows, partials, lr, beta1, beta2, weight_decay, eps, lam):
+    off = 0
+    partials.zero_()
+    for r in rows:
+        aw = r["aw"]
+        a, m1, v1, theta, drift = ref.head_step_reference(
+            aw, r["aw0"], r["dw"], r["m"], r["v"], r["step"], lr, beta1,
+            beta2, weight_decay, eps, lam, r.get("gw") if r.get("theta")
+            is not None else None, r.get("atten"))
+        aw.copy_(a)
+        r["m"].copy_(m1)
+        r["v"].copy_(v1)
+        if theta is not None:
+            r["theta"].copy_(theta)
+        partials[off] = drift
+        off += -(-aw.numel() // HEAD_STEP_CHUNK)
+
+
+@torch.no_grad()
+def head_step(rows, partials: torch.Tensor, lr: float, beta1: float,
+              beta2: float, weight_decay: float, eps: float,
+              lam: float) -> None:
+    rows = list(rows)
+    if not rows:
+        raise ValueError("head_step: empty tensor table")
+    need = head_step_partials(rows)
+    if (partials.dtype != torch.float64 or partials.numel() < need
+            or not partials.is_contiguous()
+            or partials.device != rows[0]["aw"].device):
+        raise ValueError(f"head_step: partials must be a contiguous fp64 "
+                         f"tensor of ≥ {need} entries on aw's device")
+    if not rows[0]["aw"].is_cuda:
+        torch._foreach_add_([r["step"] for r in rows], 1)
+        _head_step_cpu(rows, partials, lr, beta1, beta2, weight_decay, eps,
+                       lam)
+        return
+    ext = _ext_or_raise("head_step")
+    if ext is None:
+        raise RuntimeError("head_step has no eager GPU path")
+    table, off = [], 0
+    for r in rows:
+        table.append(_head_step_row(r, off))
+        off += -(-r["aw"].numel() // HEAD_STEP_CHUNK)
+    assert ext.head_step_chunk() == HEAD_STEP_CHUNK
+    torch._foreach_add_([r["step"] for r in rows], 1)
+    ext.head_step(table, partials.data_ptr(), partials.numel(), float(lr),
+                  float(beta1), float(beta2), float(weight_decay), float(eps),
+                  float(lam), _stream())
diff --git a/flreid_amd/ops/build.py b/flreid_amd/ops/build.py
--- a/flreid_amd/ops/build.py
+++ b/flreid_amd/ops/build.py
@@ -9,7 +9,7 @@
 CSRC = os.path.join(os.path.dirname(os.path.abspath(__file__)), "csrc")
 OUT = os.path.join(os.path.dirname(os.path.abspath(__file__)), "_flreid_hip.so")
 
-SOURCES = ["module.cpp", "elementwise.hip", "distance.hip", "window_attn.hip", "triplet.hip", "adaptive_gemm.hip", "conv3x3.hip", "conv3x3_img.hip", "conv3x3_img_ldsw.hip", "bn_train.hip", "drift.hip", "kd.hip", "patch_merge.hip", "decomposed.hip"]
+SOURCES = ["module.cpp", "elementwise.hip", "distance.hip", "window_attn.hip", "triplet.hip", "adaptive_gemm.hip", "conv3x3.hip", "conv3x3_img.hip", "conv3x3_img_ldsw.hip", "bn_train.hip", "drift.hip", "kd.hip", "patch_merge.hip", "decomposed.hip", "head_step.hip"]
 
 
 def _pybind11_includes():
diff --git a/flreid_amd/ops/csrc/adaptive_gemm.hip b/flreid_amd/ops/csrc/adaptive_gemm.hip
--- a/flreid_amd/ops/csrc/adaptive_gemm.hip
+++ b/flreid_amd/ops/csrc/adaptive_gemm.hip
@@ -14,11 +14,14 @@
 struct Prefetch {
   ushort4 xr[4];
   float4 gr[2], ar[2];
+  ushort4 tr[2];
 };
 
+template <bool PRE>
 __global__ __launch_bounds__(128) void adaptive_linear_fwd_kernel(
     const __hip_bfloat16* __restrict__ X, const float* __restrict__ GW,
     const float* __restrict__ AW, const float* __restrict__ ATTEN,
+    const __hip_bfloat16* __restrict__ TH,
     const float* __restrict__ BIAS, __hip_bfloat16* __restrict__ OUT,
     int M, int N, int K) {
   __shared__ __hip_bfloat16 lx[2][AG_BM][AG_BK + AG_PAD];
@@ -46,8 +49,12 @@
 #pragma unroll
       for (int i = 0; i < 2; ++i) {
         const int64_t base = (int64_t)(n0 + lr0 + 16 * i) * K + k0 + lc4;
-        p.gr[i] = *(const float4*)(GW + base);
-        p.ar[i] = AW ? *(const float4*)(AW + base) : float4{0.f, 0.f, 0.f, 0.f};
+        if constexpr (PRE) {
+          p.tr[i] = *(const ushort4*)(TH + base);
+        } else {
+          p.gr[i] = *(const float4*)(GW + base);
+          p.ar[i] = AW ? *(const float4*)(AW + base) : float4{0.f, 0.f, 0.f, 0.f};
+        }
       }
     } else {
 #pragma unroll
@@ -63,13 +70,19 @@
       for (int i = 0; i < 2; ++i) {
         const int nr = n0 + lr0 + 16 * i;
         float4 g = {0.f, 0.f, 0.f, 0.f}, a = {0.f, 0.f, 0.f, 0.f};
+        ushort4 th = {0, 0, 0, 0};
         if (nr < N) {
           const int64_t base = (int64_t)nr * K + k0 + lc4;
-          g = *(const float4*)(GW + base);
-          if (AW) a = *(const float4*)(AW + base);
+          if constexpr (PRE) {
+            th = *(const ushort4*)(TH + base);
+          } else {
+            g = *(const float4*)(GW + base);
+            if (AW) a = *(const float4*)(AW + base);
+          }
         }
         p.gr[i] = g;
         p.ar[i] = a;
+        p.tr[i] = th;
       }
     }
   };
@@ -82,6 +95,17 @@
       dst[1] = *(const __hip_bfloat16*)&p.xr[i].y;
       dst[2] = *(const __hip_bfloat16*)&p.xr[i].z;
       dst[3] = *(const __hip_bfloat16*)&p.xr[i].w;
+    }
+    if constexpr (PRE) {
+#pragma unroll
+      for (int i = 0; i < 2; ++i) {
+        __hip_bfloat16* dst = &lth[buf][lr0 + 16 * i][lc4];
+        dst[0] = *(const __hip_bfloat16*)&p.tr[i].x;
+        dst[1] = *(const __hip_bfloat16*)&p.tr[i].y;
+        dst[2] = *(const __hip_bfloat16*)&p.tr[i].z;
+        dst[3] = *(const __hip_bfloat16*)&p.tr[i].w;
+      }
+      return;
     }
     float at[4] = {1.f, 1.f, 1.f, 1.f};
     if (ATTEN) {
@@ -164,10 +188,30 @@
   }
   dim3 grid((M + AG_BM - 1) / AG_BM, (N + AG_BN - 1) / AG_BN);
   dim3 block(128);
-  hipLaunchKernelGGL((adaptive_linear_fwd_kernel), grid, block, 0, stream,
-                     (const __hip_bfloat16*)X, GW, AW, ATTEN, BIAS,
+  hipLaunchKernelGGL((adaptive_linear_fwd_kernel<false>), grid, block, 0,
+                     stream, (const __hip_bfloat16*)X, GW, AW, ATTEN,
+                     (const __hip_bfloat16*)nullptr, BIAS,
                      (__hip_bfloat16*)OUT, M, N, K);
   HIP_CHECK(hipGetLastError());
 }
 
-}
+extern "C" void flreid_theta_linear_fwd(const void* X, const void* TH,
+                                        const float* BIAS, void* OUT, int M,
+                                        int N, int K, hipStream_t stream) {
+  if (K % AG_BK != 0) {
+    throw std::runtime_error("theta_linear_fwd: K must be a multiple of 32");
+  }
+  if (!X || !TH || !OUT) {
+    throw std::runtime_error("theta_linear_fwd: null pointer");
+  }
+  dim3 grid((M + AG_BM - 1) / AG_BM, (N + AG_BN - 1) / AG_BN);
+  dim3 block(128);
+  hipLaunchKernelGGL((adaptive_linear_fwd_kernel<true>), grid, block, 0,
+                     stream, (const __hip_bfloat16*)X, (const float*)nullptr,
+                     (const float*)nullptr, (const float*)nullptr,
+                     (const __hip_bfloat16*)TH, BIAS, (__hip_bfloat16*)OUT,
+                     M, N, K);
+  HIP_CHECK(hipGetLastError());
+}
+
+}
diff --git a/flreid_amd/ops/csrc/head_step.hip b/flreid_amd/ops/csrc/head_step.hip
--- /dev/null
+++ b/flreid_amd/ops/csrc/head_step.hip
@@ -0,0 +1,290 @@
+
+#include "common.h"
+
+#include <vector>
+
+namespace flreid {
+
+constexpr int HS_BLOCK = 256;
+constexpr int HS_CHUNK = 1 << 14;
+constexpr int HS_MAX_TENSORS = 32;
+
+enum HeadStepFlags : int {
+  kHsGradBf16 = 1,
+  kHsVec = 2,
+  kHsTheta = 4,
+  kHsAttenVec = 8,
+};
+
+struct HeadStepTensor {
+  float* aw;
+  const float* aw0;
+  const void* dw;
+  const float* gw;
+  const float* atten;
+  float* m;
+  float* v;
+  __hip_bfloat16* theta;
+  const float* step;
+  int64_t numel;
+  int L;
+  int inner;
+  int flags;
+  int block_end;
+  int partial0;
+  int pad_;
+};
+
+struct HeadStepArgs {
+  HeadStepTensor t[HS_MAX_TENSORS];
+  double* partials;
+  double lr, beta1, beta2, weight_decay, eps;
+  float lambda;
+  int n_tensors;
+};
+static_assert(sizeof(HeadStepArgs) <= 4096, "kernel argument limit");
+
+struct HeadStepScalars {
+  double lr, beta1, beta2, weight_decay, eps;
+  float bias_correction1, bias_correction2_sqrt, lambda;
+};
+
+__device__ __forceinline__ void head_step_elem(const HeadStepScalars& s,
+                                               float& param, float aw0,
+                                               float dw, float& exp_avg,
+                                               float& exp_avg_sq,
+                                               double& drift) {
+  const float d = param - aw0;
+  drift += fabs((double)param - (double)aw0);
+  const float sgn = d > 0.f ? s.lambda : (d < 0.f ? -s.lambda : 0.f);
+  float grad = dw + sgn;
+  if (s.weight_decay != 0) {
+    grad += param * s.weight_decay;
+  }
+  exp_avg = s.beta1 * exp_avg + (1 - s.beta1) * grad;
+  exp_avg_sq = s.beta2 * exp_avg_sq + (1 - s.beta2) * grad * grad;
+  const float step_size = s.lr / s.bias_correction1;
+  float denom = (sqrtf(exp_avg_sq) / s.bias_correction2_sqrt) + s.eps;
+  param -= step_size * exp_avg / denom;
+}
+
+__device__ __forceinline__ float bf16_bits_to_float(unsigned short b) {
+  return __uint_as_float((unsigned)b << 16);
+}
+
+__global__ __launch_bounds__(HS_BLOCK) void head_step_kernel(
+    const HeadStepArgs args) {
+  int ti = 0;
+  while (ti < args.n_tensors - 1 && (int)blockIdx.x >= args.t[ti].block_end)
+    ++ti;
+  const HeadStepTensor& t = args.t[ti];
+  const int block0 = ti ? args.t[ti - 1].block_end : 0;
+  const int chunk = (int)blockIdx.x - block0;
+  const int64_t base = (int64_t)chunk * HS_CHUNK;
+  const int64_t rest = t.numel - base;
+  const int len = rest < HS_CHUNK ? (int)rest : HS_CHUNK;
+
+  HeadStepScalars s;
+  s.lr = args.lr;
+  s.beta1 = args.beta1;
+  s.beta2 = args.beta2;
+  s.weight_decay = args.weight_decay;
+  s.eps = args.eps;
+  s.lambda = args.lambda;
+  {
+    const float step_count = *t.step;
+    const double bc1 = 1 - ::pow(args.beta1, (double)step_count);
+    const double bc2 = 1 - ::pow(args.beta2, (double)step_count);
+    s.bias_correction1 = (float)bc1;
+    s.bias_correction2_sqrt = (float)::sqrt(bc2);
+  }
+
+  float* aw = t.aw + base;
+  const float* aw0 = t.aw0 + base;
+  float* m = t.m + base;
+  float* v = t.v + base;
+  const bool g16 = t.flags & kHsGradBf16;
+  const bool has_theta = t.flags & kHsTheta;
+  const float* dw32 = reinterpret_cast<const float*>(t.dw) + base;
+  const unsigned short* dw16 =
+      reinterpret_cast<const unsigned short*>(t.dw) + base;
+  const float* gw = has_theta ? t.gw + base : nullptr;
+  __hip_bfloat16* theta = has_theta ? t.theta + base : nullptr;
+  const int64_t L = t.L, inner = t.inner;
+
+  double drift = 0.0;
+
+  if (t.flags & kHsVec) {
+    const int q4 = len >> 2;
+    const bool atten_vec = t.flags & kHsAttenVec;
+#pragma unroll 2
+    for (int q = threadIdx.x; q < q4; q += HS_BLOCK) {
+      const int i0 = q << 2;
+      float4 p = *reinterpret_cast<const float4*>(aw + i0);
+      const float4 p0 = *reinterpret_cast<const float4*>(aw0 + i0);
+      float4 em = *reinterpret_cast<const float4*>(m + i0);
+      float4 ev = *reinterpret_cast<const float4*>(v + i0);
+      float4 g;
+      if (g16) {
+        const uint2 raw = *reinterpret_cast<const uint2*>(dw16 + i0);
+        g.x = __uint_as_float(raw.x << 16);
+        g.y = __uint_as_float(raw.x & 0xffff0000u);
+        g.z = __uint_as_float(raw.y << 16);
+        g.w = __uint_as_float(raw.y & 0xffff0000u);
+      } else {
+        g = *reinterpret_cast<const float4*>(dw32 + i0);
+      }
+      float4 gwv = {0.f, 0.f, 0.f, 0.f}, a4 = {0.f, 0.f, 0.f, 0.f};
+      if (has_theta) {
+        gwv = *reinterpret_cast<const float4*>(gw + i0);
+        if (atten_vec) {
+          a4 = *reinterpret_cast<const float4*>(t.atten + ((base + i0) % L));
+        } else {
+          const float a = t.atten[((base + i0) / inner) % L];
+          a4 = {a, a, a, a};
+        }
+      }
+#pragma unroll
+      for (int e = 0; e < 4; ++e) {
+        head_step_elem(s, (&p.x)[e], (&p0.x)[e], (&g.x)[e], (&em.x)[e],
+                       (&ev.x)[e], drift);
+      }
+      *reinterpret_cast<float4*>(aw + i0) = p;
+      *reinterpret_cast<float4*>(m + i0) = em;
+      *reinterpret_cast<float4*>(v + i0) = ev;
+      if (has_theta) {
+        __hip_bfloat16 th[4];
+#pragma unroll
+        for (int e = 0; e < 4; ++e) {
+          th[e] = __float2bfloat16(fmaf((&a4.x)[e], (&gwv.x)[e], (&p.x)[e]));
+        }
+        __builtin_memcpy(theta + i0, th, sizeof(th));
+      }
+    }
+    for (int i = (q4 << 2) + threadIdx.x; i < len; i += HS_BLOCK) {
+      float p = aw[i], em = m[i], ev = v[i];
+      const float g = g16 ? bf16_bits_to_float(dw16[i]) : dw32[i];
+      head_step_elem(s, p, aw0[i], g, em, ev, drift);
+      aw[i] = p;
+      m[i] = em;
+      v[i] = ev;
+      if (has_theta) {
+        const float a = t.atten[((base + i) / inner) % L];
+        theta[i] = __float2bfloat16(fmaf(a, gw[i], p));
+      }
+    }
+  } else {
+    for (int i = threadIdx.x; i < len; i += HS_BLOCK) {
+      float p = aw[i], em = m[i], ev = v[i];
+      const float g = g16 ? bf16_bits_to_float(dw16[i]) : dw32[i];
+      head_step_elem(s, p, aw0[i], g, em, ev, drift);
+      aw[i] = p;
+      m[i] = em;
+      v[i] = ev;
+      if (has_theta) {
+        const float a = t.atten[((base + i) / inner) % L];
+        theta[i] = __float2bfloat16(fmaf(a, gw[i], p));
+      }
+    }
+  }
+
+#pragma unroll
+  for (int off = 32; off > 0; off >>= 1) drift += __shfl_down(drift, off, 64);
+  __shared__ double lds[HS_BLOCK / kWave];
+  if ((threadIdx.x & (kWave - 1)) == 0) lds[threadIdx.x / kWave] = drift;
+  __syncthreads();
+  if (threadIdx.x == 0) {
+    double total = 0.0;
+#pragma unroll
+    for (int w = 0; w < HS_BLOCK / kWave; ++w) total += lds[w];
+    args.partials[t.partial0 + chunk] = total;
+  }
+}
+
+extern "C" int flreid_head_step_chunk() { return HS_CHUNK; }
+
+extern "C" void flreid_head_step(const int64_t* rows, int n_rows,
+                                 double* partials, int64_t n_partials,
+                                 double lr, double beta1, double beta2,
+                                 double weight_decay, double eps,
+                                 float lambda, hipStream_t stream) {
+  if (n_rows <= 0) throw std::runtime_error("head_step: empty tensor table");
+  if (!partials) throw std::runtime_error("head_step: null partials");
+  for (int r = 0; r < n_rows; ++r) {
+    const int64_t* row = rows + (int64_t)r * 14;
+    const int flags = (int)row[12];
+    const bool th = flags & kHsTheta;
+    const int64_t numel = row[9], L = row[10], inner = row[11];
+    const char* names[9] = {"aw", "aw0", "dw", "gw", "atten",
+                            "m",  "v",   "theta", "step"};
+    for (int k = 0; k < 9; ++k) {
+      const bool theta_only = (k == 3 || k == 4 || k == 7);
+      if (row[k] == 0 && (th || !theta_only))
+        throw std::runtime_error(std::string("head_step: null pointer '") +
+                                 names[k] + "' in row " + std::to_string(r));
+    }
+    if (numel <= 0 || L <= 0 || inner <= 0)
+      throw std::runtime_error("head_step: bad numel/L/inner in row " +
+                               std::to_string(r));
+    const int64_t nchunks = (numel + HS_CHUNK - 1) / HS_CHUNK;
+    if (row[13] < 0 || row[13] + nchunks > n_partials)
+      throw std::runtime_error("head_step: partial range out of bounds");
+    if (flags & kHsVec) {
+      const int64_t galign = (flags & kHsGradBf16) ? 8 : 16;
+      bool ok = row[0] % 16 == 0 && row[1] % 16 == 0 && row[5] % 16 == 0 &&
+                row[6] % 16 == 0 && row[2] % galign == 0;
+      if (th) {
+        ok = ok && row[3] % 16 == 0 && row[7] % 8 == 0;
+        if (flags & kHsAttenVec)
+          ok = ok && inner == 1 && L % 4 == 0 && row[4] % 16 == 0;
+        else
+          ok = ok && (L == 1 || inner % 4 == 0);
+      }
+      if (!ok)
+        throw std::runtime_error(
+            "head_step: float4 path requested for an unaligned row " +
+            std::to_string(r));
+    }
+  }
+
+  int r = 0;
+  while (r < n_rows) {
+    HeadStepArgs args;
+    int n = 0, blocks = 0;
+    for (; r < n_rows && n < HS_MAX_TENSORS; ++r, ++n) {
+      const int64_t* row = rows + (int64_t)r * 14;
+      HeadStepTensor& t = args.t[n];
+      t.aw = reinterpret_cast<float*>(row[0]);
+      t.aw0 = reinterpret_cast<const float*>(row[1]);
+      t.dw = reinterpret_cast<const void*>(row[2]);
+      t.gw = reinterpret_cast<const float*>(row[3]);
+      t.atten = reinterpret_cast<const float*>(row[4]);
+      t.m = reinterpret_cast<float*>(row[5]);
+      t.v = reinterpret_cast<float*>(row[6]);
+      t.theta = reinterpret_cast<__hip_bfloat16*>(row[7]);
+      t.step = reinterpret_cast<const float*>(row[8]);
+      t.numel = row[9];
+      t.L = (int)row[10];
+      t.inner = (int)row[11];
+      t.flags = (int)row[12];
+      t.partial0 = (int)row[13];
+      t.pad_ = 0;
+      blocks += (int)((row[9] + HS_CHUNK - 1) / HS_CHUNK);
+      t.block_end = blocks;
+    }
+    for (int k = n; k < HS_MAX_TENSORS; ++k) args.t[k] = HeadStepTensor{};
+    args.partials = partials;
+    args.lr = lr;
+    args.beta1 = beta1;
+    args.beta2 = beta2;
+    args.weight_decay = weight_decay;
+    args.eps = eps;
+    args.lambda = lambda;
+    args.n_tensors = n;
+    hipLaunchKernelGGL(head_step_kernel, dim3(blocks), dim3(HS_BLOCK), 0,
+                       stream, args);
+    HIP_CHECK(hipGetLastError());
+  }
+}
+
+}
diff --git a/flreid_amd/ops/csrc/module.cpp b/flreid_amd/ops/csrc/module.cpp
--- a/flreid_amd/ops/csrc/module.cpp
+++ b/flreid_amd/ops/csrc/module.cpp
@@ -1,7 +1,10 @@
 
 #include <pybind11/pybind11.h>
+#include <pybind11/stl.h>
 
 #include <cstdint>
+#include <stdexcept>
+#include <vector>
 
 #include <hip/hip_runtime.h>
 
@@ -99,6 +102,13 @@
                                       int64_t, int64_t, int64_t, int64_t, int,
                                       int, float, float, int, int, int,
                                       hipStream_t);
+extern "C" void flreid_theta_linear_fwd(const void*, const void*,
+                                        const float*, void*, int, int, int,
+                                        hipStream_t);
+extern "C" int flreid_head_step_chunk();
+extern "C" void flreid_head_step(const int64_t*, int, double*, int64_t,
+                                 double, double, double, double, double,
+                                 float, hipStream_t);
 }
 
 namespace py = pybind11;
@@ -398,4 +408,31 @@
               channels_last, train, lambda_l1, lambda_mask, need_aw,
               need_mask, need_atten, as_stream(stream));
         });
+
+  m.def("theta_linear_fwd",
+        [](uintptr_t x, uintptr_t theta, uintptr_t bias, uintptr_t out, int M,
+           int N, int K, uintptr_t stream) {
+          flreid::flreid_theta_linear_fwd((const void*)x, (const void*)theta,
+                                          (const float*)bias, (void*)out, M,
+                                          N, K, as_stream(stream));
+        });
+
+  m.def("head_step_chunk", []() { return flreid::flreid_head_step_chunk(); });
+
+  m.def("head_step",
+        [](const std::vector<std::vector<int64_t>>& rows, uintptr_t partials,
+           int64_t n_partials, double lr, double beta1, double beta2,
+           double weight_decay, double eps, float lambda, uintptr_t stream) {
+          std::vector<int64_t> flat;
+          flat.reserve(rows.size() * 14);
+          for (const auto& r : rows) {
+            if (r.size() != 14)
+              throw std::invalid_argument("head_step: rows need 14 fields");
+            flat.insert(flat.end(), r.begin(), r.end());
+          }
+          flreid::flreid_head_step(flat.data(), (int)rows.size(),
+                                   (double*)partials, n_partials, lr, beta1,
+                                   beta2, weight_decay, eps, lambda,
+                                   as_stream(stream));
+        });
 }
diff --git a/flreid_amd/ops/reference.py b/flreid_amd/ops/reference.py
--- a/flreid_amd/ops/reference.py
+++ b/flreid_amd/ops/reference.py
@@ -172,6 +172,34 @@
 
 
 
+def head_step_reference(aw: torch.Tensor, aw0: torch.Tensor, dw: torch.Tensor,
+                        m: torch.Tensor, v: torch.Tensor, step,
+                        lr: float, beta1: float, beta2: float,
+                        weight_decay: float, eps: float, lam: float,
+                        gw: Optional[torch.Tensor] = None,
+                        atten: Optional[torch.Tensor] = None):
+    f64 = torch.float64
+    a, a0, g = aw.detach().to(f64), aw0.detach().to(f64), dw.detach().to(f64)
+    m1, v1 = m.detach().to(f64), v.detach().to(f64)
+    lam32 = float(torch.tensor(lam, dtype=torch.float32))
+    d = a - a0
+    drift = d.abs().sum()
+    g = g + lam32 * torch.sign(d)
+    if weight_decay != 0:
+        g = g + weight_decay * a
+    m1 = beta1 * m1 + (1 - beta1) * g
+    v1 = beta2 * v1 + (1 - beta2) * g * g
+    t = float(step)
+    bc1 = 1 - beta1 ** t
+    bc2_sqrt = (1 - beta2 ** t) ** 0.5
+    a = a - (lr / bc1) * m1 / (v1.sqrt() / bc2_sqrt + eps)
+    theta = None
+    if gw is not None:
+        theta = atten.detach().to(f64) * gw.detach().to(f64) + a
+    return a, m1, v1, theta, drift
+
+
+
 def l1_hard_threshold(weights: torch.Tensor, threshold: float) -> torch.Tensor:
     return weights * torch.greater(weights.abs(), threshold).to(weights.dtype)
 
```

Measured after the change: 5087 images/sec (median of 6 runs). +17.1%, better.
